# AI4Science-WestlakeU/safediffcon

Measured on AMD Instinct MI355X. Metric: sampled control trajectories/sec (1000-step DDPM), higher is better.
Workload: dtype f32; 1 GPU; C4: 2D smoke Unet3D_with_Conv3D dim=64 (1,2,4) state (B,32,7,64,64), B=64 per GPU, guided 1000-step DDPM, conformal quantile on; batch_per_gpu=64, global_batch=64, step=U-Net + guidance + posterior update of the whole batch, one hipGraph replay, parallelism=batch-sharded x1, no data-path collective, conv_precision=fp32

## Files before the change

### include/sdc.h

```cpp
#ifndef SDC_H
#define SDC_H

#include <stddef.h>
#include <stdint.h>

#ifdef __cplusplus
extern "C" {
#endif

#define SDC_OK 0
#define SDC_EINVAL (-1)
#define SDC_EALIGN (-2)
#define SDC_EHIP (-3)
#define SDC_ENULL (-4)

int sdc_version(void);
int sdc_last_error(char* buf, size_t cap);

typedef struct SdcConvDesc {
    int32_t B, Cin0, Cin1, Cout;
    int32_t iD, iH, iW;
    int32_t oD, oH, oW;
    int32_t kD, kH, kW;
    int32_t sD, sH, sW;
    int32_t pD, pH, pW;
    int32_t uD, uH, uW;
    int32_t up_mode;
    int32_t precision;
    int64_t x0s[5], x1s[5], ys[5], rs[5];
} SdcConvDesc;

int sdc_conv(const SdcConvDesc* d, const float* x0, const float* x1, const float* wp, const float* bias,
             const float* residual, float* y, void* stream);

size_t sdc_conv_splitk_bytes(const SdcConvDesc* d);
int sdc_conv_splitk(const SdcConvDesc* d, const float* x0, const float* x1, const float* wp, const float* bias, float* y,
                    float* work, size_t work_bytes, void* stream);

int sdc_conv_describe(const SdcConvDesc* d, char* name, size_t cap, double* mfma_share);

int sdc_conv_gnparts(const SdcConvDesc* d, int G);
int sdc_conv_gn(const SdcConvDesc* d, const float* x0, const float* x1, const float* wp, const float* bias,
                const float* residual, float* y, double* parts, int G, void* stream);

int sdc_gn_stats(const float* x, float* stats, int B, int C, int G, int64_t S, float eps, void* stream);
size_t sdc_gn_stats_bytes(int B, int G);
int sdc_gn_finalize(const double* parts, float* stats, int B, int G, int nparts, int64_t n_per_group, float eps, void* stream);

int sdc_gn_apply(const float* x, const float* stats, const float* gamma, const float* beta, const float* ss,
                 const int32_t* t_dev, int64_t ss_t_stride, int64_t ss_b_stride, int64_t ss_off,
                 const float* residual, float* y, int B, int C, int G, int64_t S, void* stream);

int sdc_gn_fused_ok(int B, int C, int G, int64_t S);
int sdc_gn_fused(const float* x, const float* gamma, const float* beta, const float* ss, const int32_t* t_dev,
                 int64_t ss_t_stride, int64_t ss_b_stride, int64_t ss_off, const float* residual, float* y, int B, int C, int G,
                 int64_t S, float eps, void* stream);

int sdc_gn_pointwise_out(const float* h, const float* stats, const float* gamma, const float* beta, const float* residual,
                         const float* w, const float* bias, float* y, int B, int C, int G, int Cout, int64_t S, int64_t plane,
                         int64_t ys0, int64_t ys1, int64_t ys2, void* stream);

int sdc_chan_norm(const float* x, const float* g, const float* residual, float* y, int B, int C, int64_t S,
                  int mode, float eps, void* stream);

int sdc_linattn(const float* qkv, float* ctx, float* out, int outer, int inner, int heads, int64_t n,
                int64_t q_so, int64_t q_sc, int64_t q_si, int64_t o_so, int64_t o_sc, int64_t o_si, void* stream);

size_t sdc_linattn_block_bytes(int outer, int inner, int C, int64_t n);
int sdc_linattn_block(const float* x, const float* g_pre, const float* wqkv, const float* wo, const float* bo,
                      const float* g_post, float* work, float* y, int outer, int inner, int C, int64_t n,
                      int64_t so, int64_t sc, int64_t si, int pre_mode, int post_mode, float eps, void* stream);
int sdc_linattn_block_gn(const float* x_raw, const float* gn_stats, const float* gn_gamma, const float* gn_beta, int gn_G,
                         const float* gn_residual, const float* g_pre, const float* wqkv, const float* wo, const float* bo,
                         const float* g_post, float* work, float* y, int outer, int inner, int C, int64_t n,
                         int64_t so, int64_t sc, int64_t si, int pre_mode, int post_mode, float eps, void* stream);

int sdc_tattn_block(const float* x, const float* g_pre, const float* wqkv, const float* wo, const float* rot,
                    const float* bias, float* y, int outer, int inner, int C, int ntok, int64_t so, int64_t sc,
                    int64_t st, float eps, void* stream);

size_t sdc_pack_tattn_f16_bytes(void);
int sdc_pack_tattn_f16(const float* wqkv, const float* wo, void* dst, void* stream);
int sdc_tattn_block_f16(const float* x, const float* g_pre, const void* wpk, const float* rot, const float* bias, float* y,
                        int outer, int inner, int C, int ntok, int64_t so, int64_t sc, int64_t st, float eps, void* stream);

int sdc_attn(const float* qkv, float* out, const float* rot, const float* bias, int outer, int inner, int heads,
             int ntok, int64_t q_so, int64_t q_sc, int64_t q_si, int64_t q_st,
             int64_t o_so, int64_t o_sc, int64_t o_si, int64_t o_st, void* stream);

int sdc_act(const float* x, float* y, int64_t n, int kind, void* stream);

#define SDC_MODEL_BURGERS 0
#define SDC_MODEL_TOKAMAK 1
#define SDC_MODEL_SMOKE 2

typedef struct SdcStepDesc {
    int32_t model;
    int32_t B;
    int32_t d0, d1, d2, d3;
    int32_t guide;
    int32_t clip;
    int32_t impose;
    int32_t cond_idx;
    int32_t pad_zero;
    int32_t use_max;
    int32_t has_wgt;
    int32_t skip_draws;
    int32_t ddim;
    uint64_t seed;
} SdcStepDesc;

int sdc_guide_reduce(const SdcStepDesc* d, const float* x, const float* eps, const float* coef, const int32_t* t_dev,
                     const float* gpar, float* gscal, void* stream);
int sdc_step_update(const SdcStepDesc* d, const float* x, const float* eps, const float* gext, const float* coef,
                    const int32_t* t_dev, const int32_t* draw_dev, const float* noise, int64_t noise_stride,
                    const float* gpar, const float* gscal, const float* target, const float* c0, const float* c1,
                    const float* c2, float* xout, float* x0out, void* stream);
int sdc_impose(const SdcStepDesc* d, float* x, const float* c0, const float* c1, const float* c2, void* stream);
int sdc_randn(float* x, int64_t n, uint64_t seed, const int32_t* draw_dev, void* stream);
int sdc_advance(int32_t* t_dev, int dt, int32_t* draw_dev, int ddraw, void* stream);

int sdc_advance_table(int32_t* idx_dev, int32_t* t_dev, const int32_t* ttab, int32_t* draw_dev, int ddraw, void* stream);

int sdc_conformal_score(const SdcStepDesc* d, const float* pred, const float* truth, const float* target,
                        const float* gpar, float* score, float* weight, void* stream);

int sdc_burgers_rollout(const float* u0, const float* f, float* traj, int N, int s, int Nt, int steps, int record_every,
                        float dt, float coef_transport, float d0, float d1, float d2, void* stream);


typedef struct SdcWgradDesc {
    int32_t B, M, N;
    int32_t oD, oH, oW;
    int32_t iD, iH, iW;
    int32_t kD, kH, kW;
    int32_t sD, sH, sW;
    int32_t pD, pH, pW;
    int32_t uD, uH, uW;
    int32_t precision;
    int64_t gs[5], xs[5];
} SdcWgradDesc;
size_t sdc_conv_wgrad_bytes(const SdcWgradDesc* d);
int sdc_conv_wgrad(const SdcWgradDesc* d, const float* g, const float* x, float* dw, float* dbias, void* work,
                   size_t work_bytes, void* stream);

#define SDC_F16_EXP_INTS 1025
int sdc_f16_grad_exponent(const float* g, int B, int C, int D, int H, int W, const int64_t* strides, int32_t* e, void* stream);

int sdc_conv_dgrad_f16(const SdcConvDesc* d, const float* g, const float* wp, const int32_t* e, float* dx, void* stream);

size_t sdc_conv_wgrad_f16_bytes(const SdcWgradDesc* d);
int sdc_conv_wgrad_f16(const SdcWgradDesc* d, const float* g, const float* x, const int32_t* e, float* dw, float* dbias, void* work,
                       size_t work_bytes, void* stream);
int sdc_conv_wgrad_describe(const SdcWgradDesc* d, char* name, size_t cap);

int sdc_conv_stem_f16_ok(const SdcConvDesc* d);
size_t sdc_pack_stem_f16_bytes(int Cout, int Cin, int kD, int kH, int kW);
int sdc_pack_stem_f16(const float* w, void* out, int Cout, int Cin, int kD, int kH, int kW, void* stream);
int sdc_conv_stem_f16(const SdcConvDesc* d, const float* x, const void* wh, const float* bias, float* y, void* stream);

int sdc_conv_stem_x3_ok(const SdcConvDesc* d);
size_t sdc_pack_stem_x3_bytes(int Cout, int Cin, int kD, int kH, int kW);
int sdc_pack_stem_x3(const float* w, void* out, int Cout, int Cin, int kD, int kH, int kW, void* stream);
int sdc_conv_stem_x3(const SdcConvDesc* d, const float* x, const void* wb, const float* bias, float* y, void* stream);

int sdc_conv_gemm_x3_ok(const SdcConvDesc* d);
size_t sdc_pack_gemm_x3_bytes(int Cout, int Cin, int kH, int kW);
int sdc_pack_gemm_x3(const float* wp, void* out, int Cout, int Cin, int kH, int kW, void* stream);
int sdc_conv_gemm_x3(const SdcConvDesc* d, const float* x, const void* wb, const float* bias, float* y, void* stream);

size_t sdc_gn_silu_bwd_floats(int B, int C, int G, int64_t S);
int sdc_gn_silu_bwd(const float* h, const float* gy, const float* stats, const float* gamma, const float* beta,
                    const float* ss, int64_t ss_b_stride, float* rows, float* gh, float* dgamma, float* dbeta, float* dss,
                    int B, int C, int G, int64_t S, void* stream);

size_t sdc_chan_norm_bwd_parts(int B, int64_t S);
size_t sdc_chan_norm_bwd_bytes(int B, int C, int64_t S);
int sdc_chan_norm_bwd(const float* x, const float* gy, const float* g, float* gx, float* gpart, int B, int C, int64_t S,
                      int mode, float eps, void* stream);

size_t sdc_pack_conv_weight_floats(int Cout, int Cin, int kD, int kH, int kW, int precision);
int sdc_pack_conv_weight(const float* w, float* out, int Cout, int Cin, int kD, int kH, int kW, int precision, int flip, void* stream);

typedef struct SdcPackItem {
    const float* w;
    float* out;
    int Cout, Cin, kD, kH, kW, precision, flip;
    int co_sh, ci_sh, grid_x, grid_y, block0;
    unsigned tap_magic;
    int64_t n[5];
} SdcPackItem;
int sdc_pack_batch_plan(SdcPackItem* items, int n, int* total_blocks, int* lds_bytes);
int sdc_pack_batch_run(const SdcPackItem* items_dev, int n, int total_blocks, int lds_bytes, void* stream);

size_t sdc_attn_bwd_bytes(int outer, int inner, int heads, int ntok);
int sdc_attn_bwd(const float* qkv, const float* dout, const float* rot, const float* bias, float* dqkv, float* dbias, void* work,
                 int outer, int inner, int heads, int ntok, int64_t q_so, int64_t q_sc, int64_t q_si, int64_t q_st,
                 int64_t o_so, int64_t o_sc, int64_t o_si, int64_t o_st, void* stream);
size_t sdc_linattn_bwd_bytes(int outer, int inner, int heads, int64_t n);
int sdc_linattn_bwd(const float* qkv, const float* dout, float* dqkv, void* work, int outer, int inner, int heads, int64_t n,
                    int64_t q_so, int64_t q_sc, int64_t q_si, int64_t o_so, int64_t o_sc, int64_t o_si, void* stream);

int sdc_act_bwd(const float* x, const float* gy, float* gx, int64_t n, int kind, void* stream);

int sdc_sumpool2(const float* g, float* gx, int64_t rows, int H, int W, int fh, int fw, void* stream);

int sdc_linear(const float* x, const float* w, const float* bias, float* y, int rows, int K, int M, int64_t x_stride,
               int64_t y_stride, void* stream);
int sdc_linear_dgrad(const float* gy, const float* w, float* gx, int rows, int K, int M, int64_t gy_stride, int64_t gx_stride,
                     void* stream);
int sdc_linear_wgrad(const float* gy, const float* x, float* gw, float* gbias, int rows, int K, int M, int64_t gy_stride,
                     int64_t x_stride, void* stream);

typedef struct {
    const void* ptr;
    int64_t nwords;
} SdcSpan;
int sdc_checksum_spans(const SdcSpan* spans_dev, int n, uint64_t* out_dev, void* stream);

#define SDC_OPT_SGD 0
#define SDC_OPT_ADAM 1
#define SDC_OPT_ADAMW 2
#define SDC_OPT_CLIP 1
#define SDC_OPT_SKIP_NONFINITE 2
#define SDC_OPT_HP_LR 0
#define SDC_OPT_HP_BETA1 1
#define SDC_OPT_HP_BETA2 2
#define SDC_OPT_HP_EPS 3
#define SDC_OPT_HP_WEIGHT_DECAY 4
#define SDC_OPT_HP_MAX_GRAD_NORM 5
#define SDC_OPT_HP_EMA_BETA 6
#define SDC_OPT_HP_EMA_UPDATE_EVERY 7
#define SDC_OPT_HP_EMA_UPDATE_AFTER_STEP 8
#define SDC_OPT_HP_COUNT 9
typedef struct SdcOptItem {
    float* p;
    const float* g;
    float* m;
    float* v;
    float* ema;
    int64_t n;
    int64_t chunk0;
} SdcOptItem;
typedef struct SdcOptState {
    int64_t step;
    float grad_norm;
    float clip_coef;
    int applied;
    int ema_mode;
} SdcOptState;
int sdc_optim_plan(SdcOptItem* items, int n, int kind, int* chunk, int* total_chunks, int* grid);
size_t sdc_optim_bytes(int total_chunks);
int sdc_optim_step(int kind, const SdcOptItem* items_dev, int n, int chunk, int total_chunks, int grid, const double* hp_dev,
                   SdcOptState* state_dev, void* work, int flags, void* stream);

int sdc_graph_begin(void* stream);
int sdc_graph_end(void* stream, void** graph_exec);
int sdc_graph_launch(void* graph_exec, void* stream);
int sdc_graph_destroy(void* graph_exec);

int sdc_event_create(void** ev);
int sdc_event_record(void* ev, void* stream);
int sdc_event_elapsed_ms(void* ev0, void* ev1, float* ms);
int sdc_event_destroy(void* ev);

#define SDC_KSTAR_SEQ 10
#define SDC_KSTAR_NIN 18
#define SDC_KSTAR_UNITS 100
typedef struct {
    int nlayers;
    int width[7];
    int act[6];
    const float* params;
    int64_t stride;
} SdcKstarMlp;
typedef struct {
    int n_lstm, n_bpw;
    const float* lstm;
    int64_t lstm_stride;
    SdcKstarMlp head;
    SdcKstarMlp steady;
    SdcKstarMlp bpw;
    double lstm_ystd[4], lstm_ymean[4], nn_ystd[4], nn_ymean[4], bpw_ystd[2], bpw_ymean[2];
    double scale;
    double inputs0[15];
    double low_action[9], high_action[9];
    double year_in;
} SdcKstarModel;
size_t sdc_kstar_lstm_floats(void);
int sdc_kstar_rollout(const SdcKstarModel* m, const float* actions, int64_t act_b_stride, int64_t act_t_stride,
                      int64_t act_c_stride, double* out, double* work, int B, int nsteps, void* stream);

size_t sdc_smoke_rollout_workspace_bytes(int B);
int sdc_smoke_rollout(const float* c1, const float* c2, int64_t ctrl_b_stride, int64_t ctrl_f_stride,
                      const float* init_density, int64_t dens_b_stride, const float* init_velocity, int64_t vel_b_stride,
                      const unsigned char* fluid_mask, const unsigned char* bucket_labels, const unsigned char* safe_labels,
                      int n_buckets, int n_safe, double* out, double* out_zero, void* work, size_t work_bytes, int B, int nt,
                      int nx, int per_timelength, int ring_lo, int ring_hi, double accuracy, int max_iterations, void* stream);

#ifdef __cplusplus
}
#endif
#endif
```

### safediffcon_amd/_lib.py

```python
import ctypes as C
import os

_HERE = os.path.dirname(os.path.abspath(__file__))
LIB_PATH = os.path.join(_HERE, "libsdc_hip.so")

SDC_MODEL_BURGERS, SDC_MODEL_TOKAMAK, SDC_MODEL_SMOKE = 0, 1, 2

_f32p = C.c_void_p
_i32p = C.c_void_p
_stream = C.c_void_p
_i64 = C.c_int64


class SdcConvDesc(C.Structure):
    _fields_ = [(n, C.c_int32) for n in (
        "B", "Cin0", "Cin1", "Cout", "iD", "iH", "iW", "oD", "oH", "oW", "kD", "kH", "kW", "sD", "sH", "sW",
        "pD", "pH", "pW", "uD", "uH", "uW", "up_mode", "precision")] + [
        ("x0s", C.c_int64 * 5), ("x1s", C.c_int64 * 5), ("ys", C.c_int64 * 5), ("rs", C.c_int64 * 5)]


class SdcStepDesc(C.Structure):
    _fields_ = [(n, C.c_int32) for n in (
        "model", "B", "d0", "d1", "d2", "d3", "guide", "clip", "impose", "cond_idx", "pad_zero", "use_max",
        "has_wgt", "skip_draws", "ddim")] + [("_pad", C.c_int32), ("seed", C.c_uint64)]


class SdcWgradDesc(C.Structure):
    _fields_ = [(n, C.c_int32) for n in (
        "B", "M", "N", "oD", "oH", "oW", "iD", "iH", "iW", "kD", "kH", "kW", "sD", "sH", "sW", "pD", "pH", "pW",
        "uD", "uH", "uW", "precision")] + [("gs", C.c_int64 * 5), ("xs", C.c_int64 * 5)]


class SdcPackItem(C.Structure):
    _fields_ = [("w", C.c_void_p), ("out", C.c_void_p)] + [(n, C.c_int32) for n in (
        "Cout", "Cin", "kD", "kH", "kW", "precision", "flip", "co_sh", "ci_sh", "grid_x", "grid_y", "block0")] + [
        ("tap_magic", C.c_uint32), ("_pad", C.c_int32), ("n", C.c_int64 * 5)]


class SdcOptItem(C.Structure):
    _fields_ = [("p", C.c_void_p), ("g", C.c_void_p), ("m", C.c_void_p), ("v", C.c_void_p), ("ema", C.c_void_p),
                ("n", C.c_int64), ("chunk0", C.c_int64)]


class SdcOptState(C.Structure):
    _fields_ = [("step", C.c_int64), ("grad_norm", C.c_float), ("clip_coef", C.c_float), ("applied", C.c_int32), ("ema_mode", C.c_int32)]


class SdcSpan(C.Structure):
    _fields_ = [("ptr", C.c_void_p), ("nwords", C.c_int64)]


class SdcKstarMlp(C.Structure):
    _fields_ = [("nlayers", C.c_int32), ("width", C.c_int32 * 7), ("act", C.c_int32 * 6), ("params", C.c_void_p), ("stride", C.c_int64)]


class SdcKstarModel(C.Structure):
    _fields_ = [("n_lstm", C.c_int32), ("n_bpw", C.c_int32), ("lstm", C.c_void_p), ("lstm_stride", C.c_int64),
                ("head", SdcKstarMlp), ("steady", SdcKstarMlp), ("bpw", SdcKstarMlp),
                ("lstm_ystd", C.c_double * 4), ("lstm_ymean", C.c_double * 4), ("nn_ystd", C.c_double * 4), ("nn_ymean", C.c_double * 4),
                ("bpw_ystd", C.c_double * 2), ("bpw_ymean", C.c_double * 2), ("scale", C.c_double), ("inputs0", C.c_double * 15),
                ("low_action", C.c_double * 9), ("high_action", C.c_double * 9), ("year_in", C.c_double)]


SIGNATURES = {
    "sdc_version": (C.c_int, []),
    "sdc_last_error": (C.c_int, [C.c_char_p, C.c_size_t]),
    "sdc_conv": (C.c_int, [C.POINTER(SdcConvDesc), _f32p, _f32p, _f32p, _f32p, _f32p, _f32p, _stream]),
    "sdc_conv_describe": (C.c_int, [C.POINTER(SdcConvDesc), C.c_char_p, C.c_size_t, C.POINTER(C.c_double)]),
    "sdc_conv_gnparts": (C.c_int, [C.POINTER(SdcConvDesc), C.c_int]),
    "sdc_conv_gn": (C.c_int, [C.POINTER(SdcConvDesc), _f32p, _f32p, _f32p, _f32p, _f32p, _f32p, C.c_void_p, C.c_int, _stream]),
    "sdc_gn_finalize": (C.c_int, [C.c_void_p, _f32p, C.c_int, C.c_int, C.c_int, _i64, C.c_float, _stream]),
    "sdc_gn_stats": (C.c_int, [_f32p, _f32p, C.c_int, C.c_int, C.c_int, _i64, C.c_float, _stream]),
    "sdc_gn_stats_bytes": (C.c_size_t, [C.c_int, C.c_int]),
    "sdc_gn_apply": (C.c_int, [_f32p, _f32p, _f32p, _f32p, _f32p, _i32p, _i64, _i64, _i64, _f32p, _f32p,
                               C.c_int, C.c_int, C.c_int, _i64, _stream]),
    "sdc_gn_fused_ok": (C.c_int, [C.c_int, C.c_int, C.c_int, _i64]),
    "sdc_gn_fused": (C.c_int, [_f32p, _f32p, _f32p, _f32p, _i32p, _i64, _i64, _i64, _f32p, _f32p, C.c_int, C.c_int, C.c_int, _i64,
                               C.c_float, _stream]),
    "sdc_gn_pointwise_out": (C.c_int, [_f32p, _f32p, _f32p, _f32p, _f32p, _f32p, _f32p, _f32p, C.c_int, C.c_int, C.c_int, C.c_int, _i64,
                                       _i64, _i64, _i64, _i64, _stream]),
    "sdc_chan_norm": (C.c_int, [_f32p, _f32p, _f32p, _f32p, C.c_int, C.c_int, _i64, C.c_int, C.c_float, _stream]),
    "sdc_linattn": (C.c_int, [_f32p, _f32p, _f32p, C.c_int, C.c_int, C.c_int, _i64, _i64, _i64, _i64, _i64, _i64,
                              _i64, _stream]),
    "sdc_linattn_block_bytes": (C.c_size_t, [C.c_int, C.c_int, C.c_int, _i64]),
    "sdc_linattn_block": (C.c_int, [_f32p, _f32p, _f32p, _f32p, _f32p, _f32p, _f32p, _f32p, C.c_int, C.c_int, C.c_int, _i64,
                                    _i64, _i64, _i64, C.c_int, C.c_int, C.c_float, _stream]),
    "sdc_linattn_block_gn": (C.c_int, [_f32p, _f32p, _f32p, _f32p, C.c_int, _f32p, _f32p, _f32p, _f32p, _f32p, _f32p, _f32p, _f32p,
                                       C.c_int, C.c_int, C.c_int, _i64, _i64, _i64, _i64, C.c_int, C.c_int, C.c_float, _stream]),
    "sdc_tattn_block": (C.c_int, [_f32p, _f32p, _f32p, _f32p, _f32p, _f32p, _f32p, C.c_int, C.c_int, C.c_int, C.c_int,
                                  _i64, _i64, _i64, C.c_float, _stream]),
    "sdc_pack_tattn_f16_bytes": (C.c_size_t, []),
    "sdc_pack_tattn_f16": (C.c_int, [_f32p, _f32p, C.c_void_p, _stream]),
    "sdc_tattn_block_f16": (C.c_int, [_f32p, _f32p, C.c_void_p, _f32p, _f32p, _f32p, C.c_int, C.c_int, C.c_int, C.c_int,
                                      _i64, _i64, _i64, C.c_float, _stream]),
    "sdc_attn": (C.c_int, [_f32p, _f32p, _f32p, _f32p, C.c_int, C.c_int, C.c_int, C.c_int, _i64, _i64, _i64, _i64,
                           _i64, _i64, _i64, _i64, _stream]),
    "sdc_act": (C.c_int, [_f32p, _f32p, _i64, C.c_int, _stream]),
    "sdc_guide_reduce": (C.c_int, [C.POINTER(SdcStepDesc), _f32p, _f32p, _f32p, _i32p, _f32p, _f32p, _stream]),
    "sdc_step_update": (C.c_int, [C.POINTER(SdcStepDesc), _f32p, _f32p, _f32p, _f32p, _i32p, _i32p, _f32p, _i64,
                                  _f32p, _f32p, _f32p, _f32p, _f32p, _f32p, _f32p, _f32p, _stream]),
    "sdc_impose": (C.c_int, [C.POINTER(SdcStepDesc), _f32p, _f32p, _f32p, _f32p, _stream]),
    "sdc_randn": (C.c_int, [_f32p, _i64, C.c_uint64, _i32p, _stream]),
    "sdc_advance": (C.c_int, [_i32p, C.c_int, _i32p, C.c_int, _stream]),
    "sdc_advance_table": (C.c_int, [_i32p, _i32p, _i32p, _i32p, C.c_int, _stream]),
    "sdc_conformal_score": (C.c_int, [C.POINTER(SdcStepDesc), _f32p, _f32p, _f32p, _f32p, _f32p, _f32p, _stream]),
    "sdc_burgers_rollout": (C.c_int, [_f32p, _f32p, _f32p, C.c_int, C.c_int, C.c_int, C.c_int, C.c_int, C.c_float, C.c_float,
                                      C.c_float, C.c_float, C.c_float, _stream]),
    "sdc_conv_wgrad_bytes": (C.c_size_t, [C.POINTER(SdcWgradDesc)]),
    "sdc_conv_wgrad": (C.c_int, [C.POINTER(SdcWgradDesc), _f32p, _f32p, _f32p, _f32p, C.c_void_p, C.c_size_t, _stream]),
    "sdc_f16_grad_exponent": (C.c_int, [_f32p, C.c_int, C.c_int, C.c_int, C.c_int, C.c_int, C.c_void_p, C.c_void_p, _stream]),
    "sdc_conv_dgrad_f16": (C.c_int, [C.POINTER(SdcConvDesc), _f32p, _f32p, C.c_void_p, _f32p, _stream]),
    "sdc_conv_stem_f16_ok": (C.c_int, [C.POINTER(SdcConvDesc)]),
    "sdc_pack_stem_f16_bytes": (C.c_size_t, [C.c_int, C.c_int, C.c_int, C.c_int, C.c_int]),
    "sdc_pack_stem_f16": (C.c_int, [_f32p, C.c_void_p, C.c_int, C.c_int, C.c_int, C.c_int, C.c_int, _stream]),
    "sdc_conv_stem_f16": (C.c_int, [C.POINTER(SdcConvDesc), _f32p, C.c_void_p, _f32p, _f32p, _stream]),
    "sdc_conv_stem_x3_ok": (C.c_int, [C.POINTER(SdcConvDesc)]),
    "sdc_pack_stem_x3_bytes": (C.c_size_t, [C.c_int, C.c_int, C.c_int, C.c_int, C.c_int]),
    "sdc_pack_stem_x3": (C.c_int, [_f32p, C.c_void_p, C.c_int, C.c_int, C.c_int, C.c_int, C.c_int, _stream]),
    "sdc_conv_stem_x3": (C.c_int, [C.POINTER(SdcConvDesc), _f32p, C.c_void_p, _f32p, _f32p, _stream]),
    "sdc_conv_gemm_x3_ok": (C.c_int, [C.POINTER(SdcConvDesc)]),
    "sdc_pack_gemm_x3_bytes": (C.c_size_t, [C.c_int, C.c_int, C.c_int, C.c_int]),
    "sdc_pack_gemm_x3": (C.c_int, [_f32p, C.c_void_p, C.c_int, C.c_int, C.c_int, C.c_int, _stream]),
    "sdc_conv_gemm_x3": (C.c_int, [C.POINTER(SdcConvDesc), _f32p, C.c_void_p, _f32p, _f32p, _stream]),
    "sdc_conv_wgrad_f16_bytes": (C.c_size_t, [C.POINTER(SdcWgradDesc)]),
    "sdc_conv_wgrad_f16": (C.c_int, [C.POINTER(SdcWgradDesc), _f32p, _f32p, C.c_void_p, _f32p, _f32p, C.c_void_p, C.c_size_t, _stream]),
    "sdc_conv_wgrad_describe": (C.c_int, [C.POINTER(SdcWgradDesc), C.c_char_p, C.c_size_t]),
    "sdc_gn_silu_bwd_floats": (C.c_size_t, [C.c_int, C.c_int, C.c_int, _i64]),
    "sdc_gn_silu_bwd": (C.c_int, [_f32p, _f32p, _f32p, _f32p, _f32p, _f32p, _i64, _f32p, _f32p, _f32p, _f32p, _f32p,
                                  C.c_int, C.c_int, C.c_int, _i64, _stream]),
    "sdc_chan_norm_bwd_parts": (C.c_size_t, [C.c_int, _i64]),
    "sdc_chan_norm_bwd_bytes": (C.c_size_t, [C.c_int, C.c_int, _i64]),
    "sdc_chan_norm_bwd": (C.c_int, [_f32p, _f32p, _f32p, _f32p, _f32p, C.c_int, C.c_int, _i64, C.c_int, C.c_float, _stream]),
    "sdc_pack_conv_weight_floats": (C.c_size_t, [C.c_int, C.c_int, C.c_int, C.c_int, C.c_int, C.c_int]),
    "sdc_pack_conv_weight": (C.c_int, [_f32p, _f32p, C.c_int, C.c_int, C.c_int, C.c_int, C.c_int, C.c_int, C.c_int, _stream]),
    "sdc_pack_batch_plan": (C.c_int, [C.POINTER(SdcPackItem), C.c_int, C.POINTER(C.c_int), C.POINTER(C.c_int)]),
    "sdc_pack_batch_run": (C.c_int, [C.c_void_p, C.c_int, C.c_int, C.c_int, _stream]),
    "sdc_attn_bwd_bytes": (C.c_size_t, [C.c_int, C.c_int, C.c_int, C.c_int]),
    "sdc_attn_bwd": (C.c_int, [_f32p, _f32p, _f32p, _f32p, _f32p, _f32p, C.c_void_p, C.c_int, C.c_int, C.c_int, C.c_int,
                               _i64, _i64, _i64, _i64, _i64, _i64, _i64, _i64, _stream]),
    "sdc_linattn_bwd_bytes": (C.c_size_t, [C.c_int, C.c_int, C.c_int, _i64]),
    "sdc_linattn_bwd": (C.c_int, [_f32p, _f32p, _f32p, C.c_void_p, C.c_int, C.c_int, C.c_int, _i64, _i64, _i64, _i64, _i64, _i64, _i64,
                                  _stream]),
    "sdc_act_bwd": (C.c_int, [_f32p, _f32p, _f32p, _i64, C.c_int, _stream]),
    "sdc_sumpool2": (C.c_int, [_f32p, _f32p, _i64, C.c_int, C.c_int, C.c_int, C.c_int, _stream]),
    "sdc_kstar_lstm_floats": (C.c_size_t, []),
    "sdc_kstar_rollout": (C.c_int, [C.POINTER(SdcKstarModel), _f32p, _i64, _i64, _i64, C.c_void_p, C.c_void_p, C.c_int, C.c_int, _stream]),
    "sdc_smoke_rollout_workspace_bytes": (C.c_size_t, [C.c_int]),
    "sdc_smoke_rollout": (C.c_int, [_f32p, _f32p, _i64, _i64, _f32p, _i64, _f32p, _i64, C.c_void_p, C.c_void_p, C.c_void_p,
                                    C.c_int, C.c_int, C.c_void_p, C.c_void_p, C.c_void_p, C.c_size_t, C.c_int, C.c_int, C.c_int,
                                    C.c_int, C.c_int, C.c_int, C.c_double, C.c_int, _stream]),
    "sdc_conv_splitk_bytes": (C.c_size_t, [C.POINTER(SdcConvDesc)]),
    "sdc_conv_splitk": (C.c_int, [C.POINTER(SdcConvDesc), _f32p, _f32p, _f32p, _f32p, _f32p, _f32p, C.c_size_t, _stream]),
    "sdc_linear": (C.c_int, [_f32p, _f32p, _f32p, _f32p, C.c_int, C.c_int, C.c_int, _i64, _i64, _stream]),
    "sdc_linear_dgrad": (C.c_int, [_f32p, _f32p, _f32p, C.c_int, C.c_int, C.c_int, _i64, _i64, _stream]),
    "sdc_linear_wgrad": (C.c_int, [_f32p, _f32p, _f32p, _f32p, C.c_int, C.c_int, C.c_int, _i64, _i64, _stream]),
    "sdc_checksum_spans": (C.c_int, [C.c_void_p, C.c_int, C.c_void_p, _stream]),
    "sdc_optim_plan": (C.c_int, [C.POINTER(SdcOptItem), C.c_int, C.c_int, C.POINTER(C.c_int), C.POINTER(C.c_int), C.POINTER(C.c_int)]),
    "sdc_optim_bytes": (C.c_size_t, [C.c_int]),
    "sdc_optim_step": (C.c_int, [C.c_int, C.c_void_p, C.c_int, C.c_int, C.c_int, C.c_int, C.c_void_p, C.c_void_p, C.c_void_p, C.c_int,
                                 _stream]),
    "sdc_graph_begin": (C.c_int, [_stream]),
    "sdc_graph_end": (C.c_int, [_stream, C.POINTER(C.c_void_p)]),
    "sdc_graph_launch": (C.c_int, [C.c_void_p, _stream]),
    "sdc_graph_destroy": (C.c_int, [C.c_void_p]),
    "sdc_event_create": (C.c_int, [C.POINTER(C.c_void_p)]),
    "sdc_event_record": (C.c_int, [C.c_void_p, _stream]),
    "sdc_event_elapsed_ms": (C.c_int, [C.c_void_p, C.c_void_p, C.POINTER(C.c_float)]),
    "sdc_event_destroy": (C.c_int, [C.c_void_p]),
}

_lib = None


class SdcError(RuntimeError):
    pass


def use_library(path):
    global LIB_PATH
    if _lib is not None:
        raise SdcError("use_library() after the library has been loaded")
    LIB_PATH = os.path.abspath(path)


def get_lib():
    global _lib
    if _lib is None:
        if not os.path.exists(LIB_PATH):
            raise SdcError(
                f"{LIB_PATH} not found: build it with `python -m safediffcon_amd.build` "
                "(hipcc --offload-arch=gfx950). safediffcon_amd has no CPU/eager fallback.")
        lib = C.CDLL(LIB_PATH)
        for name, (res, args) in SIGNATURES.items():
            fn = getattr(lib, name)
            fn.restype, fn.argtypes = res, args
        _lib = lib
    return _lib


def last_error():
    buf = C.create_string_buffer(512)
    get_lib().sdc_last_error(buf, 512)
    return buf.value.decode(errors="replace")


def check(rc, what=""):
    if rc != 0:
        raise SdcError(f"{what or 'libsdc_hip'} failed (code {rc}): {last_error()}")
```

### safediffcon_amd/build.py

```python
import os
import subprocess
import sys

HERE = os.path.dirname(os.path.abspath(__file__))
CSRC = os.path.join(HERE, "csrc")
LIB = os.path.join(HERE, "libsdc_hip.so")
SOURCES = ["sdc_api.hip", "sdc_conv.hip", "sdc_conv_wino.hip", "sdc_conv_f16.hip", "sdc_conv_stem_f16.hip", "sdc_conv_stem_x3.hip", "sdc_conv_gemm_x3.hip", "sdc_norm.hip", "sdc_attn.hip", "sdc_lablock.hip", "sdc_tablock.hip", "sdc_tablock_f16.hip", "sdc_step.hip", "sdc_solver.hip", "sdc_grad.hip", "sdc_wgrad_f16.hip", "sdc_attn_bwd.hip", "sdc_kstar.hip", "sdc_smoke.hip", "sdc_linear.hip", "sdc_optim.hip"]
HEADERS = ["sdc_common.h", "sdc_conv.h", "sdc_conv_wino3s.inc", "sdc_conv_wino2s.inc", "sdc_conv_pw2.inc"]
HIPCC = os.environ.get("HIPCC", "/opt/rocm/bin/hipcc")
FLAGS = ["--offload-arch=gfx950", "-O3", "-fPIC", "-std=c++17", "-Wall", "-Wno-unused-function"]


def source_hash():
    import hashlib
    h = hashlib.sha256()
    for f in SOURCES + HEADERS:
        with open(os.path.join(CSRC, f), "rb") as fh:
            h.update(fh.read())
    with open(os.path.join(HERE, "..", "include", "sdc.h"), "rb") as fh:
        h.update(fh.read())
    return h.hexdigest()[:16]


def _stale(out, deps):
    if not os.path.exists(out):
        return True
    t = os.path.getmtime(out)
    return any(os.path.getmtime(d) > t for d in deps)


def build_experiments(verbose=True):
    out = os.path.join(HERE, "libsdc_hip_exp.so")
    cmd = [HIPCC, *FLAGS, "-DSDC_KERNEL_EXPERIMENTS", "-shared", *[os.path.join(CSRC, s) for s in SOURCES], "-o", out]
    if verbose:
        print(" ".join(cmd), flush=True)
    subprocess.check_call(cmd)
    return out


def build(force=False, verbose=True, jobs=4):
    from concurrent.futures import ThreadPoolExecutor
    hdrs = [os.path.join(CSRC, h) for h in HEADERS] + [os.path.join(HERE, "..", "include", "sdc.h")]
    objs, todo = [], []
    for src in SOURCES:
        s = os.path.join(CSRC, src)
        o = os.path.join(CSRC, src.replace(".hip", ".o"))
        if force or _stale(o, [s] + hdrs):
            todo.append([HIPCC, *FLAGS, "-c", s, "-o", o])
        objs.append(o)

    def run(cmd):
        if verbose:
            print(" ".join(cmd), flush=True)
        subprocess.check_call(cmd)
    if todo:
        with ThreadPoolExecutor(max_workers=max(1, min(jobs, len(todo)))) as ex:
            list(ex.map(run, todo))
    if force or _stale(LIB, objs):
        run([HIPCC, "--offload-arch=gfx950", "-shared", "-fPIC", *objs, "-o", LIB])
    return LIB


if __name__ == "__main__":
    if "--experiments" in sys.argv:
        build_experiments()
    else:
        build(force="--force" in sys.argv)
```

### safediffcon_amd/engine.py

```python
import ctypes as C
import functools
import os
import math

import torch

from . import _lib
from ._lib import SdcConvDesc, check


def _ptr(t):
    return 0 if t is None else t.data_ptr()


def _s5(t):
    assert t.dim() == 5, t.shape
    return tuple(int(s) for s in t.stride())


def as5(t):
    while t.dim() < 5:
        t = t.unsqueeze(2)
    return t


@functools.lru_cache(maxsize=16)
def _up2_merge(parity, device):
    return torch.tensor([[1, 0, 0], [0, 1, 1]] if parity == 0 else [[1, 1, 0], [0, 0, 1]], dtype=torch.float64, device=device)


def pack_conv_weight(t, kind="conv", precision=0):
    def base():
        if kind == "convT":
            t5 = as5(t)
            t5 = t5.flip(2, 3, 4).permute(2, 3, 4, 0, 1)
            return t5.reshape(-1, t5.shape[-1]).contiguous()
        if isinstance(kind, tuple) and kind[0] == "convT_sub":
            _, ph, pw = kind
            t5 = as5(t)
            kh = (3, 1) if ph == 0 else (2, 0)
            kw = (3, 1) if pw == 0 else (2, 0)
            sub = t5[:, :, 0][:, :, (1 - ph)::2][:, :, :, (1 - pw)::2].flip(2, 3)
            assert kh == ((3, 1) if ph == 0 else (2, 0)) and kw == ((3, 1) if pw == 0 else (2, 0))
            return sub.permute(2, 3, 0, 1).reshape(-1, sub.shape[1]).contiguous()
        if isinstance(kind, tuple) and kind[0] == "up2_sub":
            _, ph, pw = kind
            t5 = as5(t).to(torch.float64)
            mh, mw = _up2_merge(ph, t5.device), _up2_merge(pw, t5.device)
            sub = torch.einsum("ah,bw,oihw->oiab", mh, mw, t5[:, :, 0])
            return sub.permute(2, 3, 1, 0).reshape(-1, sub.shape[0]).to(torch.float32).contiguous()
        if kind == "unshuffle":
            co, c4 = t.shape[0], t.shape[1]
            t4 = t.reshape(co, c4 // 4, 2, 2)
            return t4.permute(2, 3, 1, 0).reshape(-1, co).contiguous()
        t5 = as5(t)
        return t5.permute(2, 3, 4, 1, 0).reshape(-1, t5.shape[0]).contiguous()
    if precision in (6, 7):
        p4 = pack_conv_weight(t, kind, 4)
        k = tuple(as5(t).shape[2:])
        if kind != "conv" or f16_kc(k) == 0:
            return p4
        return torch.cat([p4, p4.new_zeros(-p4.numel() % 4), f16_tail(t)])
    wp = base().to(torch.float32)
    if precision not in (2, 3, 4, 5) or kind != "conv" or t.shape[-1] != 3:
        return wp
    t5 = as5(t).to(torch.float64)
    G = torch.tensor([[1, 0, 0], [.5, .5, .5], [.5, -.5, .5], [0, 0, 1]], dtype=torch.float64, device=t5.device)
    u = torch.einsum("xk,oidhk->dhxio", G, t5)
    parts = [wp.reshape(-1), u.reshape(-1).to(torch.float32)]
    if precision == 5 and t5.shape[2] == 1 and t5.shape[3] == 1:
        G43 = torch.tensor([[1 / 4, 0, 0], [-1 / 6, -1 / 6, -1 / 6], [-1 / 6, 1 / 6, -1 / 6], [1 / 24, 1 / 12, 1 / 6],
                            [1 / 24, -1 / 12, 1 / 6], [0, 0, 1]], dtype=torch.float64, device=t5.device)
        u43 = torch.einsum("xk,oik->xio", G43, t5[:, :, 0, 0])
        return torch.cat(parts + [u43.reshape(-1).to(torch.float32)])
    if precision >= 3 and t5.shape[3] == 3:
        u2 = torch.einsum("jh,xk,oidhk->diojx", G, G, t5)
        parts.append(u2.reshape(-1).to(torch.float32))
        if precision >= 4 and t5.shape[2] == 3:
            u3 = torch.einsum("zd,jh,xk,oidhk->ziojx", G, G, G, t5)
            parts.append(u3.reshape(-1).to(torch.float32))
    return torch.cat(parts)


def f16_kc(k):
    k = tuple(k)
    return 32 if tuple(k) in ((1, 1, 3), (1, 3, 3), (3, 3, 3)) else 0


def f16_tail(t, flip=False):
    t5 = as5(t).to(torch.float32)
    if flip:
        t5 = t5.transpose(0, 1).flip((2, 3, 4))
    co, ci = t5.shape[0], t5.shape[1]
    kc = f16_kc(t5.shape[2:])
    nch = (ci + kc - 1) // kc
    w = t5.permute(2, 3, 4, 1, 0).reshape(-1, ci, co)
    w = torch.cat([w, w.new_zeros(w.shape[0], nch * kc - ci, co)], 1)
    w = w.reshape(w.shape[0], nch, kc, co).permute(0, 1, 3, 2).contiguous()
    return w.half().reshape(-1).view(torch.float32)


def pack_stem_f16(w):
    t5 = as5(w).to(torch.float32)
    co, ci, kD, kH, kW = t5.shape
    if not (kW == 7 and (kD, kH) in ((1, 1), (1, 7), (7, 7)) and 1 <= ci <= 8):
        raise ValueError(f"pack_stem_f16: taps 1x1x7, 1x7x7 or 7x7x7 and Cin <= 8 (got {tuple(t5.shape)})")
    taps, ns = kH * 7, (kH * 7 + 1) // 2
    z = t5.new_zeros(co, 8, kD, 2 * ns)
    z[:, :ci, :, :taps] = t5.reshape(co, ci, kD, taps)
    z = z.reshape(co, 8, kD, ns, 2).permute(2, 3, 0, 4, 1).contiguous()
    return z.half().reshape(-1).view(torch.float32)


def pack_stem_x3(w):
    t5 = as5(w).to(torch.float32)
    co, ci, kD, kH, kW = t5.shape
    if not (kW == 7 and (kD, kH) in ((1, 1), (1, 7), (7, 7)) and 1 <= ci <= 8):
        raise ValueError(f"pack_stem_x3: taps 1x1x7, 1x7x7 or 7x7x7 and Cin <= 8 (got {tuple(t5.shape)})")
    taps, ns = kH * 7, (kH * 7 + 1) // 2
    z = t5.new_zeros(co, 8, kD, 2 * ns)
    z[:, :ci, :, :taps] = t5.reshape(co, ci, kD, taps)
    z = z.reshape(co, 8, kD, ns, 2).permute(2, 3, 0, 4, 1).contiguous()
    return torch.stack(split3_bf16(z)).reshape(-1).view(torch.float32)


def pack_tattn_f16(wqkv, wo):
    wqkv, wo = wqkv.to(torch.float32), wo.to(torch.float32)
    if tuple(wqkv.shape) != (384, 64) or tuple(wo.shape) != (64, 128):
        raise ValueError(f"pack_tattn_f16: to_qkv (384, 64) and to_out (64, 128) (got {tuple(wqkv.shape)}, {tuple(wo.shape)})")
    a = wqkv.reshape(3, 4, 32, 4, 2, 8).permute(1, 0, 3, 4, 2, 5)
    b = wo.reshape(2, 32, 4, 2, 2, 2, 4).permute(2, 0, 3, 5, 1, 4, 6)
    return torch.cat([a.reshape(-1), b.reshape(-1)]).half().view(torch.float32)


def pack_gemm_x3(wp, cout, cin, k):
    k = tuple(k)[-2:]
    ncb = {(4, 4): 1, (2, 2): 2, (1, 1): 4}.get(k, 0)
    taps = k[0] * k[1]
    if ncb == 0 or cout <= 0 or cout % 64 or cin <= 0 or cin % (16 * ncb) or tuple(wp.shape) != (taps * cin, cout):
        raise ValueError(f"pack_gemm_x3: taps 4x4, 2x2 or 1x1, Cout % 64 == 0, Cin % {16 * max(ncb, 1)} == 0, Wp [taps * Cin][Cout] "
                         f"(got taps {k}, Cin {cin}, Cout {cout}, Wp {tuple(wp.shape)})")
    z = wp.to(torch.float32).reshape(taps, cin // (16 * ncb), ncb, 16, cout // 64, 64)
    z = z.permute(4, 1, 2, 0, 5, 3).contiguous()
    return torch.stack(split3_bf16(z)).reshape(-1).view(torch.float32)


def split3_bf16(x):
    h = x.bfloat16()
    r = x - h.float()
    m = r.bfloat16()
    return h, m, (r - m.float()).bfloat16()


def conv_precision(n, k, cin, cout, f16=None, train=False):
    floats = functools.partial(_lib.get_lib().sdc_pack_conv_weight_floats, cout, cin, *k)
    if train:
        assert f16 in (6, 7) and n == floats(8), (f16, n, k, cin, cout)
        return f16
    if f16 in (6, 7) and f16_kc(k) > 0 and n == floats(6):
        return f16
    code = next((p for p in (0, 2, 3, 4, 5) if n == floats(p)), None)
    assert code is not None, (n, k, cin, cout)
    return code


def conv_desc(x, x1, out, residual, cout, k, stride, pad, up, up_mode, precision):
    d = SdcConvDesc()
    d.B, d.Cin0, d.iD, d.iH, d.iW = x.shape
    d.Cin1, d.Cout = (0 if x1 is None else x1.shape[1]), cout
    d.oD, d.oH, d.oW = out.shape[2:]
    d.kD, d.kH, d.kW = k
    d.sD, d.sH, d.sW = stride
    d.pD, d.pH, d.pW = pad
    d.uD, d.uH, d.uW = up
    d.up_mode, d.precision = up_mode, precision
    d.x0s[:] = _s5(x)
    d.x1s[:] = _s5(x1) if x1 is not None else (0,) * 5
    d.ys[:] = _s5(out)
    d.rs[:] = _s5(residual) if residual is not None else (0,) * 5
    return d


class Pool:

    def __init__(self, device):
        self.device = device
        self.free = {}
        self.all = []
        self.bytes = 0

    def get(self, shape):
        n = int(math.prod(shape))
        lst = self.free.get(n)
        if lst:
            return lst.pop().view(shape)
        t = torch.empty(n, dtype=torch.float32, device=self.device)
        self.all.append(t)
        self.bytes += n * 4
        return t.view(shape)

    def put(self, t):
        self.free.setdefault(t.numel(), []).append(t.reshape(-1))


class Plan:

    def __init__(self, device, precision=0, stem_f16=False, stem_split=False, gemm_split=False, attn_f16=False):
        self.device = torch.device(device)
        self.lib = _lib.get_lib()
        self.precision = int(precision)
        if self.precision not in (0, 2, 3, 4, 5, 6, 7):
            raise ValueError(f"precision must be 0, 2, 3, 4, 5, 6 or 7 (got {precision})")
        self.stem_f16 = bool(stem_f16)
        self.stem_split = bool(stem_split) and self.precision >= 4 and not self.stem_f16
        self.gemm_split = bool(gemm_split) and self.precision >= 4
        self.attn_f16 = bool(attn_f16)
        self.calls = []
        self.pool = Pool(self.device)
        self.keep = []
        self.repackers = []
        self._stats = None
        self._ctx = None
        self._gn_parts = {}
        self.fuse_gn_stats = True
        self.fuse_gn_small = True
        self.split_small_grids = False

    def run(self, stream):
        for fn, args in self.calls:
            rc = fn(*args, stream)
            if rc:
                check(rc, fn.__name__)

    def refresh_weights(self):
        with torch.no_grad():
            for dst, fn in self.repackers:
                dst.copy_(fn())

    def _stats_buf(self, B, G):
        need = int(self.lib.sdc_gn_stats_bytes(B, G))
        if self._stats is None or self._stats.numel() * 4 < need:
            self._stats = torch.empty((need + 3) // 4, dtype=torch.float32, device=self.device)
            self.keep.append(self._stats)
        return self._stats

    def _ctx_buf(self, n):
        if self._ctx is None or self._ctx.numel() < n:
            self._ctx = torch.empty(n, dtype=torch.float32, device=self.device)
            self.keep.append(self._ctx)
        return self._ctx

    def _emit(self, fn, *args):
        self.calls.append((fn, args))

    def packed(self, src_fn):
        with torch.no_grad():
            w = src_fn().detach().to(self.device, torch.float32).contiguous().clone()
        self.repackers.append((w, lambda: src_fn().detach().to(self.device, torch.float32)))
        self.keep.append(w)
        return w

    def conv_weight(self, w, kind="conv"):
        return self.packed(lambda: pack_conv_weight(w() if callable(w) else w, kind, self.precision))

    def stem_weight(self, w, pack=pack_stem_f16):
        return self.packed(lambda: pack(w() if callable(w) else w))

    def vec(self, p):
        return self.packed(lambda: (p() if callable(p) else p).reshape(-1))

    def conv(self, x, wp, bias, cout, k, *, x1=None, stride=(1, 1, 1), pad=(0, 0, 0), up=(1, 1, 1), up_mode=0,
             residual=None, out=None, gn_groups=0, stem_w=None, gemm_w=None):
        B, c0, iD, iH, iW = x.shape
        c1 = 0 if x1 is None else x1.shape[1]

        def osz(i, u, kk, s, p):
            v = (i - 1) * u + 1 if up_mode else i * u
            return (v + 2 * p - kk) // s + 1

        o = tuple(osz(i, u, kk, s, p) for i, u, kk, s, p in zip((iD, iH, iW), up, k, stride, pad))
        if out is None:
            out = self.pool.get((B, cout, *o))
        else:
            assert tuple(out.shape[:2]) == (B, cout) and out.dim() == 5, (out.shape, (B, cout, *o))
            o = tuple(out.shape[2:])
        if (self.stem_f16 or self.stem_split) and stem_w is not None and x1 is None and residual is None:
            d = conv_desc(x, None, out, None, cout, k, stride, pad, up, up_mode, 0)
            ok, fn, pack = ((self.lib.sdc_conv_stem_f16_ok, self.lib.sdc_conv_stem_f16, pack_stem_f16) if self.stem_f16 else
                            (self.lib.sdc_conv_stem_x3_ok, self.lib.sdc_conv_stem_x3, pack_stem_x3))
            if ok(C.byref(d)):
                wh = self.stem_weight(stem_w, pack)
                self.keep += [d, x, wh, bias, out]
                self._emit(fn, C.byref(d), _ptr(x), _ptr(wh), _ptr(bias), _ptr(out))
                return out
        if self.gemm_split and gemm_w is not None and x1 is None and residual is None and not gn_groups:
            d = conv_desc(x, None, out, None, cout, k, stride, pad, up, up_mode, 0)
            if self.lib.sdc_conv_gemm_x3_ok(C.byref(d)) and not (self.split_small_grids and self.lib.sdc_conv_splitk_bytes(C.byref(d))):
                wb = self.packed(lambda: pack_gemm_x3(gemm_w(), cout, c0, k))
                self.keep += [d, x, wb, bias, out]
                self._emit(self.lib.sdc_conv_gemm_x3, C.byref(d), _ptr(x), _ptr(wb), _ptr(bias), _ptr(out))
                return out
        if callable(wp):
            wp = wp()
        prec = conv_precision(wp.numel(), k, c0 + c1, cout, f16=self.precision)
        d = conv_desc(x, x1, out, residual, cout, k, stride, pad, up, up_mode, prec)
        if residual is not None:
            assert tuple(residual.shape) == tuple(out.shape)
        self.keep += [d, x, x1, wp, bias, residual, out]
        if self.split_small_grids and residual is None:
            nsplit = int(self.lib.sdc_conv_splitk_bytes(C.byref(d)))
            if nsplit:
                work = torch.empty(nsplit // 4, dtype=torch.float32, device=self.device)
                self.keep.append(work)
                self._emit(self.lib.sdc_conv_splitk, C.byref(d), _ptr(x), _ptr(x1), _ptr(wp), _ptr(bias), _ptr(out), _ptr(work), nsplit)
                return out
        nparts = int(self.lib.sdc_conv_gnparts(C.byref(d), gn_groups)) if (gn_groups and self.fuse_gn_stats) else 0
        if nparts > 0:
            parts = torch.empty(B * gn_groups * nparts * 2, dtype=torch.float64, device=self.device)
            self.keep.append(parts)
            self._gn_parts[out.data_ptr()] = (parts, nparts, gn_groups)
            self._emit(self.lib.sdc_conv_gn, C.byref(d), _ptr(x), _ptr(x1), _ptr(wp), _ptr(bias), _ptr(residual), _ptr(out),
                       _ptr(parts), gn_groups)
            return out
        self._emit(self.lib.sdc_conv, C.byref(d), _ptr(x), _ptr(x1), _ptr(wp), _ptr(bias), _ptr(residual), _ptr(out))
        return out

    def conv_transpose_422(self, x, w, bias, cout):
        B, c0, iD, iH, iW = x.shape
        out = self.pool.get((B, cout, iD, 2 * iH, 2 * iW))
        for ph in (0, 1):
            for pw in (0, 1):
                kind = ("convT_sub", ph, pw)
                if self.gemm_split:
                    self.conv(x, lambda kind=kind: self.conv_weight(w, kind), bias, cout, (1, 2, 2), pad=(0, 1 - ph, 1 - pw),
                              out=out[:, :, :, ph::2, pw::2], gemm_w=lambda kind=kind: pack_conv_weight(w() if callable(w) else w, kind, 0))
                    continue
                wp = self.conv_weight(w, kind)
                self.conv(x, wp, bias, cout, (1, 2, 2), pad=(0, 1 - ph, 1 - pw), out=out[:, :, :, ph::2, pw::2])
        return out

    def upsample2_conv3(self, x, w, bias, cout):
        B, c0, iD, iH, iW = x.shape
        out = self.pool.get((B, cout, iD, 2 * iH, 2 * iW))
        for ph in (0, 1):
            for pw in (0, 1):
                wp = self.conv_weight(w, ("up2_sub", ph, pw))
                self.conv(x, wp, bias, cout, (1, 2, 2), pad=(0, 1 - ph, 1 - pw), out=out[:, :, :, ph::2, pw::2])
        return out

    def gn_silu(self, x, gamma, beta, groups, *, ss=None, t_dev=None, ss_t_stride=0, ss_b_stride=0, ss_off=0,
                residual=None, out=None, eps=1e-5):
        assert x.is_contiguous()
        B, Cc = x.shape[0], x.shape[1]
        S = x.numel() // (B * Cc)
        st = self._stats_buf(B, groups)
        out = x if out is None else out
        self.keep += [x, gamma, beta, ss, t_dev, residual, out]
        fused = self._gn_parts.pop(x.data_ptr(), None)
        if fused is not None and fused[2] == groups:
            self._emit(self.lib.sdc_gn_finalize, _ptr(fused[0]), _ptr(st), B, groups, fused[1], (Cc // groups) * S, eps)
        elif self.fuse_gn_small and self.lib.sdc_gn_fused_ok(B, Cc, groups, S):
            self._emit(self.lib.sdc_gn_fused, _ptr(x), _ptr(gamma), _ptr(beta), _ptr(ss), _ptr(t_dev), ss_t_stride, ss_b_stride,
                       ss_off, _ptr(residual), _ptr(out), B, Cc, groups, S, eps)
            return out
        else:
            self._emit(self.lib.sdc_gn_stats, _ptr(x), _ptr(st), B, Cc, groups, S, eps)
        self._emit(self.lib.sdc_gn_apply, _ptr(x), _ptr(st), _ptr(gamma), _ptr(beta), _ptr(ss), _ptr(t_dev),
                   ss_t_stride, ss_b_stride, ss_off, _ptr(residual), _ptr(out), B, Cc, groups, S)
        return out

    def chan_norm(self, x, g, mode, *, residual=None, out=None, eps=1e-5):
        assert x.is_contiguous()
        B, Cc = x.shape[0], x.shape[1]
        S = x.numel() // (B * Cc)
        if out is None:
            out = self.pool.get(tuple(x.shape))
        self.keep += [x, g, residual, out]
        self._emit(self.lib.sdc_chan_norm, _ptr(x), _ptr(g), _ptr(residual), _ptr(out), B, Cc, S, mode, eps)
        return out

    def act(self, x, kind, out=None):
        out = x if out is None else out
        self.keep += [x, out]
        self._emit(self.lib.sdc_act, _ptr(x), _ptr(out), x.numel(), kind)
        return out

    def linattn(self, qkv, heads, outer, inner, n, q_strides, out, o_strides):
        ctx = self._ctx_buf(outer * inner * heads * 32 * 32)
        self.keep += [qkv, out]
        self._emit(self.lib.sdc_linattn, _ptr(qkv), _ptr(ctx), _ptr(out), outer, inner, heads, n, *q_strides, *o_strides)
        return out

    def gn_stats_deferred(self, x, groups, eps=1e-5):
        assert x.is_contiguous()
        B, Cc = x.shape[0], x.shape[1]
        S = x.numel() // (B * Cc)
        st = torch.empty((int(self.lib.sdc_gn_stats_bytes(B, groups)) + 3) // 4, dtype=torch.float32, device=self.device)
        self.keep += [x, st]
        fused = self._gn_parts.pop(x.data_ptr(), None)
        if fused is not None and fused[2] == groups:
            self._emit(self.lib.sdc_gn_finalize, _ptr(fused[0]), _ptr(st), B, groups, fused[1], (Cc // groups) * S, eps)
        else:
            self._emit(self.lib.sdc_gn_stats, _ptr(x), _ptr(st), B, Cc, groups, S, eps)
        return st

    def gn_apply_deferred(self, x, gn):
        st, gamma, beta, groups, res = gn
        B, Cc = x.shape[0], x.shape[1]
        S = x.numel() // (B * Cc)
        self.keep += [x, st, gamma, beta, res]
        self._emit(self.lib.sdc_gn_apply, _ptr(x), _ptr(st), _ptr(gamma), _ptr(beta), 0, 0, 0, 0, 0, _ptr(res), _ptr(x), B, Cc, groups, S)
        return x

    def gn_pointwise_out(self, x, gn, w, bias, out):
        st, gamma, beta, groups, res = gn
        B, Cc = x.shape[0], x.shape[1]
        S = x.numel() // (B * Cc)
        cout = out.shape[1]
        plane = out.shape[3] * out.shape[4]
        ys = _s5(out)
        ok = (x.is_contiguous() and (res is None or res.is_contiguous()) and cout <= 16 and Cc % 4 == 0 and Cc <= 2048 and S >= 1024 and plane % 4 == 0 and ys[4] == 1 and
              ys[3] == out.shape[4] and all(v % 4 == 0 for v in ys[:3]) and out.data_ptr() % 16 == 0 and
              tuple(out.shape[2:]) == tuple(x.shape[2:]))
        if not ok:
            return None
        self.keep += [x, st, gamma, beta, res, w, bias, out]
        self._emit(self.lib.sdc_gn_pointwise_out, _ptr(x), _ptr(st), _ptr(gamma), _ptr(beta), _ptr(res), _ptr(w), _ptr(bias), _ptr(out),
                   B, Cc, groups, cout, S, plane, ys[0], ys[1], ys[2])
        return out

    def linattn_block(self, x, g_pre, wqkv, wo, bo, g_post, outer, inner, n, strides, pre_mode, post_mode, eps=1e-5, gn=None):
        Cc = x.shape[1]
        y = self.pool.get(tuple(x.shape))
        work = torch.empty(int(self.lib.sdc_linattn_block_bytes(outer, inner, Cc, n)) // 4, dtype=torch.float32, device=self.device)
        self.keep += [x, g_pre, wqkv, wo, bo, g_post, work, y]
        if gn is not None:
            st, gamma, beta, groups, res = gn
            assert outer == x.shape[0] and (res is None or (tuple(res.shape) == tuple(x.shape) and res.stride() == x.stride()))
            self.keep += [st, gamma, beta, res]
            self._emit(self.lib.sdc_linattn_block_gn, _ptr(x), _ptr(st), _ptr(gamma), _ptr(beta), groups, _ptr(res), _ptr(g_pre),
                       _ptr(wqkv), _ptr(wo), _ptr(bo), _ptr(g_post), _ptr(work), _ptr(y), outer, inner, Cc, n, *strides, pre_mode,
                       post_mode, eps)
            return y
        self._emit(self.lib.sdc_linattn_block, _ptr(x), _ptr(g_pre), _ptr(wqkv), _ptr(wo), _ptr(bo), _ptr(g_post), _ptr(work),
                   _ptr(y), outer, inner, Cc, n, *strides, pre_mode, post_mode, eps)
        return y

    def tattn_weight(self, wqkv, wo):
        return self.packed(lambda: pack_tattn_f16(wqkv() if callable(wqkv) else wqkv, wo() if callable(wo) else wo))

    def tattn_block(self, x, g_pre, wqkv, wo, rot, bias, eps=1e-5):
        B, Cc, Fr, H, W = x.shape
        assert x.is_contiguous()
        y = self.pool.get(tuple(x.shape))
        if self.attn_f16:
            wpk = self.tattn_weight(wqkv, wo)
            self.keep += [x, g_pre, wpk, rot, bias, y]
            self._emit(self.lib.sdc_tattn_block_f16, _ptr(x), _ptr(g_pre), _ptr(wpk), _ptr(rot), _ptr(bias), _ptr(y),
                       B, H * W, Cc, Fr, Cc * Fr * H * W, Fr * H * W, H * W, eps)
            return y
        self.keep += [x, g_pre, wqkv, wo, rot, bias, y]
        self._emit(self.lib.sdc_tattn_block, _ptr(x), _ptr(g_pre), _ptr(wqkv), _ptr(wo), _ptr(rot), _ptr(bias), _ptr(y),
                   B, H * W, Cc, Fr, Cc * Fr * H * W, Fr * H * W, H * W, eps)
        return y

    def attn(self, qkv, out, heads, outer, inner, ntok, q_strides, o_strides, rot=None, bias=None):
        self.keep += [qkv, out, rot, bias]
        self._emit(self.lib.sdc_attn, _ptr(qkv), _ptr(out), _ptr(rot), _ptr(bias), outer, inner, heads, ntok,
                   *q_strides, *o_strides)
        return out
```

### safediffcon_amd/unet.py

```python
import ctypes as C
import functools
import math
import os

import torch
from torch import nn

from ._lib import check, get_lib
from .engine import Plan, as5, pack_conv_weight

HEADS, DIM_HEAD = 4, 32
HID = HEADS * DIM_HEAD


def _resnet_spec(p, cin, cout, time_dim, k):
    s = []
    if time_dim is not None:
        s += [(f"{p}.mlp.1.weight", (cout * 2, time_dim)), (f"{p}.mlp.1.bias", (cout * 2,))]
    for blk, ci in (("block1", cin), ("block2", cout)):
        s += [(f"{p}.{blk}.proj.weight", (cout, ci, *k)), (f"{p}.{blk}.proj.bias", (cout,)),
              (f"{p}.{blk}.norm.weight", (cout,)), (f"{p}.{blk}.norm.bias", (cout,))]
    if cin != cout:
        s += [(f"{p}.res_conv.weight", (cout, cin, *([1] * len(k)))), (f"{p}.res_conv.bias", (cout,))]
    return s


def spec_lucid(dim, dim_mults, channels, nd):
    one, k3, k7 = [1] * nd, [3] * nd, [7] * nd
    g = (1, 0, *one)
    td = dim * 4
    dims = [dim] + [dim * m for m in dim_mults]
    io = list(zip(dims[:-1], dims[1:]))
    gshape = lambda c: (1, c, *one)
    s = []
    if nd == 1:
        s += [("init_conv.weight", (dim, channels, *k7)), ("init_conv.bias", (dim,))]
    s += [("time_mlp.1.weight", (td, dim)), ("time_mlp.1.bias", (td,)),
          ("time_mlp.3.weight", (td, td)), ("time_mlp.3.bias", (td,))]
    if nd == 2:
        s += [("init_conv.weight", (dim, channels, *k7)), ("init_conv.bias", (dim,))]

    def lin_attn(p, c):
        return [(f"{p}.fn.fn.to_qkv.weight", (HID * 3, c, *one)), (f"{p}.fn.fn.to_out.0.weight", (c, HID, *one)),
                (f"{p}.fn.fn.to_out.0.bias", (c,)), (f"{p}.fn.fn.to_out.1.g", gshape(c)), (f"{p}.fn.norm.g", gshape(c))]

    def full_attn(p, c):
        return [(f"{p}.fn.fn.to_qkv.weight", (HID * 3, c, *one)), (f"{p}.fn.fn.to_out.weight", (c, HID, *one)),
                (f"{p}.fn.fn.to_out.bias", (c,)), (f"{p}.fn.norm.g", gshape(c))]

    downs, ups = [], []
    for i, (ci, co) in enumerate(io):
        last = i == len(io) - 1
        p = f"downs.{i}"
        downs += _resnet_spec(f"{p}.0", ci, ci, td, k3) + _resnet_spec(f"{p}.1", ci, ci, td, k3) + lin_attn(f"{p}.2", ci)
        if last:
            downs += [(f"{p}.3.weight", (co, ci, *k3)), (f"{p}.3.bias", (co,))]
        elif nd == 2:
            downs += [(f"{p}.3.1.weight", (co, ci * 4, *one)), (f"{p}.3.1.bias", (co,))]
        else:
            downs += [(f"{p}.3.weight", (co, ci, 4)), (f"{p}.3.bias", (co,))]
    mid = dims[-1]
    mids = _resnet_spec("mid_block1", mid, mid, td, k3) + full_attn("mid_attn", mid) + _resnet_spec("mid_block2", mid, mid, td, k3)
    for i, (ci, co) in enumerate(reversed(io)):
        last = i == len(io) - 1
        p = f"ups.{i}"
        ups += _resnet_spec(f"{p}.0", co + ci, co, td, k3) + _resnet_spec(f"{p}.1", co + ci, co, td, k3) + lin_attn(f"{p}.2", co)
        if last:
            ups += [(f"{p}.3.weight", (ci, co, *k3)), (f"{p}.3.bias", (ci,))]
        else:
            ups += [(f"{p}.3.1.weight", (ci, co, *k3)), (f"{p}.3.1.bias", (ci,))]
    fin = _resnet_spec("final_res_block", dim * 2, dim, td, k3) + [("final_conv.weight", (channels, dim, *one)),
                                                                   ("final_conv.bias", (channels,))]
    if nd == 2:
        return s + downs + mids + ups + fin
    return s + downs + ups + mids + fin


def spec_smoke(dim, dim_mults, channels):
    td = dim * 4
    dims = [dim] + [dim * m for m in dim_mults]
    io = list(zip(dims[:-1], dims[1:]))
    k3, one = (3, 3, 3), (1, 1, 1)
    rot = ("rotary_emb.freqs", (DIM_HEAD // 2,))

    def t_attn(p, c):
        return [(f"{p}.fn.fn.fn.{rot[0]}", rot[1]), (f"{p}.fn.fn.fn.to_qkv.weight", (HID * 3, c)),
                (f"{p}.fn.fn.fn.to_out.weight", (c, HID)), (f"{p}.fn.norm.gamma", (1, c, 1, 1, 1))]

    def s_lin(p, c):
        return [(f"{p}.fn.fn.to_qkv.weight", (HID * 3, c, 1, 1)), (f"{p}.fn.fn.to_out.weight", (c, HID, 1, 1)),
                (f"{p}.fn.fn.to_out.bias", (c,)), (f"{p}.fn.norm.gamma", (1, c, 1, 1, 1))]

    s = [("time_rel_pos_bias.relative_attention_bias.weight", (32, HEADS)),
         ("init_conv.weight", (dim, channels, 7, 7, 7)), ("init_conv.bias", (dim,))]
    s += t_attn("init_temporal_attn", dim)
    s += [("time_mlp.1.weight", (td, dim)), ("time_mlp.1.bias", (td,)), ("time_mlp.3.weight", (td, td)),
          ("time_mlp.3.bias", (td,))]
    downs, ups = [], []
    for i, (ci, co) in enumerate(io):
        p = f"downs.{i}"
        downs += _resnet_spec(f"{p}.0", ci, co, td, k3) + _resnet_spec(f"{p}.1", co, co, td, k3) + s_lin(f"{p}.2", co) + t_attn(f"{p}.3", co)
        if i < len(io) - 1:
            downs += [(f"{p}.4.weight", (co, co, 1, 4, 4)), (f"{p}.4.bias", (co,))]
    for i, (ci, co) in enumerate(reversed(io)):
        p = f"ups.{i}"
        ups += _resnet_spec(f"{p}.0", co * 2, ci, td, k3) + _resnet_spec(f"{p}.1", ci, ci, td, k3) + s_lin(f"{p}.2", ci) + t_attn(f"{p}.3", ci)
        if i < len(io) - 1:
            ups += [(f"{p}.4.weight", (ci, ci, 1, 4, 4)), (f"{p}.4.bias", (ci,))]
    mid = dims[-1]
    mids = _resnet_spec("mid_block1", mid, mid, td, k3)
    mids += [("mid_spatial_attn.fn.fn.fn.to_qkv.weight", (HID * 3, mid)), ("mid_spatial_attn.fn.fn.fn.to_out.weight", (mid, HID)),
             ("mid_spatial_attn.fn.norm.gamma", (1, mid, 1, 1, 1))]
    mids += t_attn("mid_temporal_attn", mid) + _resnet_spec("mid_block2", mid, mid, td, k3)
    fin = _resnet_spec("final_conv.0", dim * 2, dim, None, k3) + [("final_conv.1.weight", (channels, dim, *one)),
                                                                 ("final_conv.1.bias", (channels,))]
    return s + downs + ups + mids + fin


def _register(root, key, value):
    *mods, leaf = key.split(".")
    m = root
    for name in mods:
        if name not in m._modules:
            m.add_module(name, nn.Module())
        m = m._modules[name]
    m.register_parameter(leaf, nn.Parameter(value))


def _default_init(spec, gen):
    out = {}
    for key, shape in spec:
        leaf = key.rsplit(".", 1)[-1]
        if key.endswith("rotary_emb.freqs"):
            d = 2 * shape[0]
            v = 1.0 / (10000 ** (torch.arange(0, d, 2)[: d // 2].float() / d))
        elif key.endswith("relative_attention_bias.weight"):
            v = torch.randn(shape, generator=gen)
        elif leaf in ("g", "gamma") or key.endswith("norm.weight"):
            v = torch.ones(shape)
        elif key.endswith("norm.bias"):
            v = torch.zeros(shape)
        else:
            wshape = shape if leaf != "bias" else None
            if wshape is None:
                wkey = key[: -len("bias")] + "weight"
                wshape = dict(spec)[wkey]
            bound = 1.0 / math.sqrt(max(1, math.prod(wshape[1:])))
            v = (torch.rand(shape, generator=gen) * 2 - 1) * bound
        out[key] = v
    return out


def sinusoid_table(times, dim, theta=10000.0):
    return _sinusoid(times.detach().cpu(), dim, theta)


@functools.lru_cache(maxsize=32)
def _sinusoid_freqs(n, device, theta):
    return torch.exp(torch.arange(n) * -(math.log(theta) / (n - 1))).to(device)


def _sinusoid(t, dim, theta=10000.0):
    half = dim // 2
    f = _sinusoid_freqs(half, t.device, theta)
    a = t[:, None] * f[None, :]
    if dim % 2 == 0:
        return torch.cat((a.sin(), a.cos()), dim=-1)
    half1 = (dim + 1) // 2
    f1 = _sinusoid_freqs(half1, t.device, theta)
    return torch.cat((a.sin(), (t[:, None] * f1[None, :]).cos()), dim=-1)


class _Builder:

    def __init__(self, net, plan):
        self.net, self.plan = net, plan
        self.cond_sites = []

    def W(self, key, kind="conv"):
        return self.plan.conv_weight(lambda: self.net.P(key), kind)

    def V(self, key):
        return self.plan.vec(lambda: self.net.P(key))

    def ksize(self, key):
        shp = tuple(self.net.P(key).shape[2:])
        return (1,) * (3 - len(shp)) + shp

    def conv(self, x, prefix, *, x1=None, stride=1, pad=None, up=(1, 1, 1), residual=None, out=None, kind="conv",
             bias=True, gn_groups=0):
        wkey = f"{prefix}.weight"
        w = self.net.P(wkey)
        if kind == "convT":
            cout, k = w.shape[1], self.ksize(wkey)
        elif kind == "unshuffle":
            cout, k = w.shape[0], (1, 2, 2)
        else:
            cout, k = w.shape[0], self.ksize(wkey)
        if isinstance(stride, int):
            stride = tuple(stride if kk > 1 else 1 for kk in k)
        if pad is None:
            pad = tuple(kk // 2 for kk in k)
        b = self.V(f"{prefix}.bias") if bias else None
        if (self.plan.stem_f16 or self.plan.stem_split) and kind == "conv" and k[2] == 7:
            return self.plan.conv(x, lambda: self.W(wkey, kind), b, cout, k, x1=x1, stride=stride, pad=pad, up=up, residual=residual,
                                  out=out, gn_groups=gn_groups, stem_w=lambda: self.net.P(wkey))
        if self.plan.gemm_split and kind == "conv" and k in ((1, 4, 4), (1, 1, 1)) and x1 is None and residual is None:
            return self.plan.conv(x, lambda: self.W(wkey, kind), b, cout, k, stride=stride, pad=pad, up=up, out=out, gn_groups=gn_groups,
                                  gemm_w=lambda: pack_conv_weight(self.net.P(wkey), kind, 0))
        return self.plan.conv(x, self.W(wkey, kind), b, cout, k, x1=x1, stride=stride, pad=pad, up=up,
                              up_mode=1 if kind == "convT" else 0, residual=residual, out=out, gn_groups=gn_groups)

    def final_conv(self, res_prefix, conv_prefix, h, groups, x1, out):
        pool = self.plan.pool
        if self.net.fuse_final_conv and h.shape[2] * h.shape[3] * h.shape[4] >= 1024:
            g, gn, rbuf = self.resnet(res_prefix, h, groups, x1=x1, defer_gn=True)
            wv, bv = self.V(f"{conv_prefix}.weight"), self.V(f"{conv_prefix}.bias")
            if self.plan.gn_pointwise_out(g, gn, wv, bv, out) is not None:
                pool.put(g)
                if rbuf is not None:
                    pool.put(rbuf)
                return
            self.plan.gn_apply_deferred(g, gn)
            if rbuf is not None:
                pool.put(rbuf)
            f = g
        else:
            f = self.resnet(res_prefix, h, groups, x1=x1)
        self.conv(f, conv_prefix, out=out)
        pool.put(f)

    def gn(self, x, prefix, groups, residual=None, cond_off=None):
        self.plan.gn_silu(x, self.V(f"{prefix}.weight"), self.V(f"{prefix}.bias"), groups, residual=residual)
        if cond_off is not None:
            self.cond_sites.append((len(self.plan.calls) - 1, cond_off))

    def resnet(self, prefix, x, groups, *, x1=None, defer_gn=False):
        net, pool = self.net, self.plan.pool
        h = self.conv(x, f"{prefix}.block1.proj", x1=x1, gn_groups=groups)
        self.gn(h, f"{prefix}.block1.norm", groups, cond_off=net.cond_offsets.get(prefix))
        g = self.conv(h, f"{prefix}.block2.proj", gn_groups=groups)
        pool.put(h)
        own = net.has(f"{prefix}.res_conv.weight")
        if own:
            r = self.conv(x, f"{prefix}.res_conv", x1=x1)
        else:
            assert x1 is None
            r = x
        if defer_gn:
            st = self.plan.gn_stats_deferred(g, groups)
            return g, (st, self.V(f"{prefix}.block2.norm.weight"), self.V(f"{prefix}.block2.norm.bias"), groups, r), (r if own else None)
        self.gn(g, f"{prefix}.block2.norm", groups, residual=r)
        if own:
            pool.put(r)
        return g


class _HipUNet(nn.Module):

    def __init__(self, spec, dim, seed=None):
        super().__init__()
        gen = torch.Generator()
        gen.manual_seed(int(torch.initial_seed()) & 0x7FFFFFFF if seed is None else seed)
        for k, v in _default_init(spec, gen).items():
            _register(self, k, v)
        self._spec = spec
        self._plans = {}
        self.precision = 4
        self.train_precision = None
        self.stem_f16 = False
        self.attn_f16 = False
        self.stem_split = True
        self.gemm_split = True
        self.fuse_linattn = True
        self.fuse_gn_into_linattn = True
        self.content_stamp = True
        self.subpixel_upsample = True
        self.split_small_grids = False
        self.fuse_final_conv = True
        self.forward_graph = True
        self._side = None
        self.dim = dim
        self.self_condition = False
        self.cond_offsets, off = {}, 0
        for k, shape in spec:
            if k.endswith(".mlp.1.weight"):
                self.cond_offsets[k[: -len(".mlp.1.weight")]] = off
                off += shape[0]
        self.cond_width = off

    @property
    def train_precision(self):
        return self.__dict__.get("_train_precision")

    @train_precision.setter
    def train_precision(self, v):
        from .autograd import check_train_precision
        self.__dict__["_train_precision"] = check_train_precision(v)

    def P(self, key):
        m = self
        *mods, leaf = key.split(".")
        for name in mods:
            m = m._modules[name]
        return m._parameters[leaf]

    def has(self, key):
        try:
            return self.P(key) is not None
        except KeyError:
            return False

    def _trainer(self):
        if getattr(self, "_train_ctx", None) is None:
            from .autograd import Trainer
            self._train_ctx = Trainer(self)
        return self._train_ctx

    def forward_train(self, x, time):
        if not x.is_cuda:
            raise RuntimeError("safediffcon_amd runs on MI355X only: tensors must be on a cuda (HIP) device; "
                               "there is no CPU fallback")
        from . import autograd
        fn = autograd.forward_train_smoke if isinstance(self, Unet3D_with_Conv3D) else autograd.forward_train_lucid
        with self._trainer().step(x.device):
            return fn(self, x.to(torch.float32), time)

    def _drop_plans(self):
        self._train_ctx = None
        for e in self._plans.values():
            g = e.get("graph")
            if g is not None:
                torch.cuda.synchronize(e["x"].device)
                e["plan"].lib.sdc_graph_destroy(g)
                e["graph"] = None
        self._plans = {}
        self._side = None

    def _apply(self, fn, *a, **k):
        self._drop_plans()
        return super()._apply(fn, *a, **k)

    def load_state_dict(self, sd, strict=True, **kw):
        sd = {k: v for k, v in sd.items() if ("rotary_emb." not in k) or k.endswith("rotary_emb.freqs")}
        r = super().load_state_dict(sd, strict=strict, **kw)
        self.refresh()
        return r

    def _stamp_tensors(self):
        return [t for t in list(self.parameters()) + list(self.buffers()) if t.is_cuda and t.numel() and t.element_size() == 4]

    def _content_stamp(self):
        ts = self._stamp_tensors()
        if not ts:
            return 0
        from ._lib import SdcSpan
        dev = ts[0].device
        key = tuple((t.data_ptr(), t.numel()) for t in ts)
        tab = getattr(self, "_span_tab", None)
        if tab is None or tab[0] != key:
            arr = (SdcSpan * len(ts))(*[SdcSpan(t.data_ptr(), t.numel()) for t in ts])
            host = torch.frombuffer(bytearray(bytes(arr)), dtype=torch.uint8)
            tab = self._span_tab = (key, host.to(dev), torch.zeros(1, dtype=torch.int64, device=dev))
        lib = get_lib()
        check(lib.sdc_checksum_spans(tab[1].data_ptr(), len(ts), tab[2].data_ptr(), torch.cuda.current_stream(dev).cuda_stream),
              "sdc_checksum_spans")
        return int(tab[2].item())

    def _weights_stamp(self):
        host = hash(tuple((p.data_ptr(), p._version) for p in self.parameters()))
        dev = next(self.parameters()).device
        if not (self.content_stamp and dev.type == "cuda"):
            return (host, 0)
        if torch.cuda.is_current_stream_capturing():
            return (host, getattr(self, "_last_content", 0))
        self._last_content = self._content_stamp()
        return (host, self._last_content)

    def _refresh_entry(self, e, stamp):
        e["plan"].refresh_weights()
        e["cond"].refresh_weights()
        e["lut_valid"] = False
        e["wstamp"] = stamp

    def refresh(self):
        stamp = self._weights_stamp()
        for e in self._plans.values():
            self._refresh_entry(e, stamp)

    def device(self):
        return next(self.parameters()).device

    def entry(self, shape, rows, lut=False):
        key = (tuple(shape), rows, bool(lut), int(self.precision), bool(self.fuse_linattn), bool(self.subpixel_upsample),
               bool(self.fuse_gn_into_linattn), bool(self.split_small_grids), bool(self.fuse_final_conv), bool(self.stem_f16),
               bool(self.stem_split), bool(self.gemm_split), bool(self.attn_f16))
        stamp = self._weights_stamp()
        ent = self._plans.get(key)
        if ent is not None and ent["wstamp"] != stamp:
            self._refresh_entry(ent, stamp)
        if key not in self._plans:
            dev = self.device()
            if dev.type != "cuda":
                raise RuntimeError("safediffcon_amd runs on MI355X only: move the model to a cuda (HIP) device; "
                                   "there is no CPU fallback")
            plan = Plan(dev, precision=self.precision, stem_f16=bool(self.stem_f16), stem_split=bool(self.stem_split),
                        gemm_split=bool(self.gemm_split), attn_f16=bool(self.attn_f16))
            plan.split_small_grids = bool(self.split_small_grids)
            x = torch.zeros(shape, dtype=torch.float32, device=dev)
            eps = torch.zeros(shape, dtype=torch.float32, device=dev)
            b = _Builder(self, plan)
            self._build(b, x, eps)
            plan.cond_sites = b.cond_sites
            cond = Plan(dev)
            td = self.dim * 4
            emb = torch.zeros((rows, self.dim, 1, 1, 1), dtype=torch.float32, device=dev)
            cb = _Builder(self, cond)
            h = cb.conv(emb, "time_mlp.1")
            cond.act(h, 1)
            temb = cb.conv(h, "time_mlp.3")
            cond.act(temb, 0)
            prefixes = list(self.cond_offsets)
            wcat = cond.conv_weight(lambda: torch.cat([self.P(f"{p}.mlp.1.weight") for p in prefixes], 0))
            bcat = cond.vec(lambda: torch.cat([self.P(f"{p}.mlp.1.bias") for p in prefixes], 0))
            ss = cond.conv(temb, wcat, bcat, self.cond_width, (1, 1, 1))
            assert temb.shape[1] == td
            self._plans[key] = dict(plan=plan, cond=cond, x=x, eps=eps, emb=emb, ss=ss, rows=rows, lut_valid=False,
                                    t_dev=None, wstamp=stamp)
        return self._plans[key]

    def bind_cond(self, ent, t_dev):
        plan, ss, W = ent["plan"], ent["ss"], self.cond_width
        for idx, off in plan.cond_sites:
            fn, a = plan.calls[idx]
            a = list(a)
            i0 = 3 if fn is plan.lib.sdc_gn_fused else 4
            if t_dev is None:
                a[i0:i0 + 5] = ss.data_ptr(), 0, 0, W, off
            else:
                a[i0:i0 + 5] = ss.data_ptr(), t_dev.data_ptr(), W, 0, off
            plan.calls[idx] = (fn, tuple(a))
        ent["t_dev"] = t_dev

    def fill_cond(self, ent, times, stream):
        ent["emb"].copy_(sinusoid_table(times, self.dim).reshape(ent["emb"].shape), non_blocking=False)
        ent["cond"].run(stream)

    def forward(self, x, time, x_self_cond=None, **unused):
        if not x.is_cuda:
            raise RuntimeError("safediffcon_amd runs on MI355X only: tensors must be on a cuda (HIP) device; "
                               "there is no CPU fallback")
        ent = self.entry(tuple(x.shape), x.shape[0])
        stream = torch.cuda.current_stream(x.device).cuda_stream
        with torch.no_grad():
            if not ent.get("bound"):
                self.bind_cond(ent, None)
                ent["bound"] = True
            ent["x"].copy_(x)
            emb = _sinusoid(time.detach().to(x.device), self.dim)
            ent["emb"].copy_(emb.reshape(ent["emb"].shape))
            if not self.forward_graph:
                ent["cond"].run(stream)
                ent["plan"].run(stream)
                return ent["eps"].clone()
            cur = torch.cuda.current_stream(x.device)
            if self._side is None or self._side.device != x.device:
                self._side = torch.cuda.Stream(x.device)
            side = self._side
            side.wait_stream(cur)
            lib = ent["plan"].lib
            if ent.get("graph") is None:
                check(lib.sdc_graph_begin(side.cuda_stream), "sdc_graph_begin")
                try:
                    ent["cond"].run(side.cuda_stream)
                    ent["plan"].run(side.cuda_stream)
                finally:
                    g = C.c_void_p()
                    rc = lib.sdc_graph_end(side.cuda_stream, C.byref(g))
                check(rc, "sdc_graph_end")
                ent["graph"] = g
            check(lib.sdc_graph_launch(ent["graph"], side.cuda_stream), "sdc_graph_launch")
            cur.wait_stream(side)
            return ent["eps"].clone()


class _LucidUNet(_HipUNet):
    ND = 2
    NORM_MODE = 0

    def __init__(self, dim, init_dim=None, out_dim=None, dim_mults=(1, 2, 4, 8), channels=3, self_condition=False,
                 resnet_block_groups=8, learned_variance=False, learned_sinusoidal_cond=False,
                 random_fourier_features=False, learned_sinusoidal_dim=16, sinusoidal_pos_emb_theta=10000,
                 attn_dim_head=32, attn_heads=4, condition_on_residual=None):
        unsupported = dict(init_dim=init_dim, out_dim=out_dim, self_condition=self_condition or None,
                           learned_variance=learned_variance or None,
                           learned_sinusoidal_cond=learned_sinusoidal_cond or None,
                           random_fourier_features=random_fourier_features or None,
                           condition_on_residual=condition_on_residual)
        bad = [k for k, v in unsupported.items() if v is not None]
        if bad or attn_dim_head != 32 or attn_heads != 4 or sinusoidal_pos_emb_theta != 10000:
            raise NotImplementedError(f"options never enabled by the reference configs are not built: {bad}")
        super().__init__(spec_lucid(dim, tuple(dim_mults), channels, self.ND), dim)
        self.channels, self.dim_mults, self.groups = channels, tuple(dim_mults), resnet_block_groups
        self.out_dim = channels
        self.random_or_learned_sinusoidal_cond = False

    def _lin_attn(self, b, prefix, x):
        plan, pool = b.plan, b.plan.pool
        B, C = x.shape[0], x.shape[1]
        n = x.numel() // (B * C)
        if self.fuse_linattn and C in (64, 128) and n % 64 == 0:
            return plan.linattn_block(x, b.V(f"{prefix}.fn.norm.g"), b.W(f"{prefix}.fn.fn.to_qkv.weight"),
                                      b.W(f"{prefix}.fn.fn.to_out.0.weight"), b.V(f"{prefix}.fn.fn.to_out.0.bias"),
                                      b.V(f"{prefix}.fn.fn.to_out.1.g"), B, 1, n, (C * n, n, 0), self.NORM_MODE, self.NORM_MODE)
        xn = plan.chan_norm(x, b.V(f"{prefix}.fn.norm.g"), self.NORM_MODE)
        qkv = b.conv(xn, f"{prefix}.fn.fn.to_qkv", bias=False)
        pool.put(xn)
        o = pool.get((B, HID, *x.shape[2:]))
        plan.linattn(qkv, HEADS, B, 1, n, (3 * HID * n, n, 0), o, (HID * n, n, 0))
        pool.put(qkv)
        y = b.conv(o, f"{prefix}.fn.fn.to_out.0")
        pool.put(o)
        plan.chan_norm(y, b.V(f"{prefix}.fn.fn.to_out.1.g"), self.NORM_MODE, residual=x, out=y)
        return y

    def _full_attn(self, b, prefix, x):
        plan, pool = b.plan, b.plan.pool
        B, C = x.shape[0], x.shape[1]
        n = x.numel() // (B * C)
        xn = plan.chan_norm(x, b.V(f"{prefix}.fn.norm.g"), self.NORM_MODE)
        qkv = b.conv(xn, f"{prefix}.fn.fn.to_qkv", bias=False)
        pool.put(xn)
        o = pool.get((B, HID, *x.shape[2:]))
        plan.attn(qkv, o, HEADS, B, 1, n, (3 * HID * n, n, 0, 1), (HID * n, n, 0, 1))
        pool.put(qkv)
        y = b.conv(o, f"{prefix}.fn.fn.to_out", residual=x)
        pool.put(o)
        return y

    def _build(self, b, x, eps):
        pool, G = b.plan.pool, self.groups
        nres = len(self.dim_mults)
        x5, e5 = as5(x), as5(eps)
        h = b.conv(x5, "init_conv")
        r = h
        hs = []
        for i in range(nres):
            p = f"downs.{i}"
            x1 = b.resnet(f"{p}.0", h, G)
            if h is not r:
                pool.put(h)
            hs.append(x1)
            x2 = b.resnet(f"{p}.1", x1, G)
            x3 = self._lin_attn(b, f"{p}.2", x2)
            pool.put(x2)
            hs.append(x3)
            h = self._down(b, f"{p}.3", x3, i == nres - 1)
        m = b.resnet("mid_block1", h, G)
        pool.put(h)
        a = self._full_attn(b, "mid_attn", m)
        pool.put(m)
        h = b.resnet("mid_block2", a, G)
        pool.put(a)
        for i in range(nres):
            p = f"ups.{i}"
            s = hs.pop()
            y1 = b.resnet(f"{p}.0", h, G, x1=s)
            pool.put(h), pool.put(s)
            s = hs.pop()
            y2 = b.resnet(f"{p}.1", y1, G, x1=s)
            pool.put(y1), pool.put(s)
            y3 = self._lin_attn(b, f"{p}.2", y2)
            pool.put(y2)
            h = self._up(b, f"{p}.3", y3, i == nres - 1)
            pool.put(y3)
        b.final_conv("final_res_block", "final_conv", h, G, r, e5)
        pool.put(h), pool.put(r)


class Unet2D(_LucidUNet):
    ND, NORM_MODE = 2, 0

    def _down(self, b, p, x, last):
        if last:
            return b.conv(x, p)
        return b.conv(x, f"{p}.1", kind="unshuffle", stride=(1, 2, 2), pad=(0, 0, 0))

    def _up(self, b, p, x, last):
        if last:
            return b.conv(x, p)
        if self.subpixel_upsample:
            return b.plan.upsample2_conv3(x, lambda p=p: self.P(f"{p}.1.weight"), b.V(f"{p}.1.bias"), self.P(f"{p}.1.weight").shape[0])
        return b.conv(x, f"{p}.1", up=(1, 2, 2))


class Unet1D(_LucidUNet):
    ND, NORM_MODE = 1, 1

    def __init__(self, dim, init_dim=None, out_dim=None, dim_mults=(1, 2, 4, 8), channels=12, **kw):
        super().__init__(dim, init_dim, out_dim, dim_mults, channels, **kw)

    def _down(self, b, p, x, last):
        if last:
            return b.conv(x, p)
        return b.conv(x, p, stride=(1, 1, 2), pad=(0, 0, 1))

    def _up(self, b, p, x, last):
        if last:
            return b.conv(x, p)
        return b.conv(x, f"{p}.1", up=(1, 1, 2))


def rel_pos_bias_table(weight, n, num_buckets=32, max_distance=32):
    q = torch.arange(n)
    rel = q[None, :] - q[:, None]
    m = -rel
    nb = num_buckets // 2
    ret = (m < 0).long() * nb
    m = m.abs()
    max_exact = nb // 2
    small = m < max_exact
    large = max_exact + (torch.log(m.float() / max_exact) / math.log(max_distance / max_exact) * (nb - max_exact)).long()
    large = torch.min(large, torch.full_like(large, nb - 1))
    bucket = (ret + torch.where(small, m, large)).to(weight.device)
    return weight[bucket].permute(2, 0, 1).contiguous()


class Unet3D_with_Conv3D(_HipUNet):

    def __init__(self, dim, cond_dim=None, out_dim=None, dim_mults=(1, 2, 4, 8), channels=6, attn_heads=4,
                 attn_dim_head=32, use_bert_text_cond=False, init_dim=None, init_kernel_size=7,
                 use_sparse_linear_attn=True, block_type="resnet", resnet_groups=8):
        if (cond_dim is not None or out_dim is not None or use_bert_text_cond or init_dim is not None
                or init_kernel_size != 7 or not use_sparse_linear_attn or attn_heads != 4 or attn_dim_head != 32):
            raise NotImplementedError("options never enabled by the reference's 2D scripts are not built")
        super().__init__(spec_smoke(dim, tuple(dim_mults), channels), dim)
        self.channels, self.dim_mults, self.groups = channels, tuple(dim_mults), resnet_groups
        self.has_cond = False
        shared = self.P("init_temporal_attn.fn.fn.fn.rotary_emb.freqs")
        shared.requires_grad_(False)
        for k, _ in self._spec:
            if k.endswith("rotary_emb.freqs"):
                m = self
                for name in k.split(".")[:-1]:
                    m = m._modules[name]
                m._parameters["freqs"] = shared

    def _attn_tables(self, b, F):
        plan = b.plan
        if not hasattr(plan, "_rot"):
            def rot():
                fr = self.P("init_temporal_attn.fn.fn.fn.rotary_emb.freqs").detach().float().cpu()
                ang = torch.arange(F, dtype=torch.float32)[:, None] * fr[None, :]
                return torch.stack((ang.cos(), ang.sin()), dim=-1).reshape(-1)
            plan._rot = plan.packed(rot)
            plan._bias = plan.packed(lambda: rel_pos_bias_table(
                self.P("time_rel_pos_bias.relative_attention_bias.weight").detach(), F).reshape(-1))
        return plan._rot, plan._bias

    def _temporal(self, b, prefix, x):
        plan, pool = b.plan, b.plan.pool
        B, C, F, H, W = x.shape
        hw = H * W
        rot, bias = self._attn_tables(b, F)
        if self.fuse_linattn and C == 64 and F == 32 and hw % 8 == 0 and x.is_contiguous():
            if plan.attn_f16:
                return plan.tattn_block(x, b.V(f"{prefix}.fn.norm.gamma"), lambda: self.P(f"{prefix}.fn.fn.fn.to_qkv.weight"),
                                        lambda: self.P(f"{prefix}.fn.fn.fn.to_out.weight"), rot, bias)
            return plan.tattn_block(x, b.V(f"{prefix}.fn.norm.gamma"), b.W(f"{prefix}.fn.fn.fn.to_qkv.weight"),
                                    b.W(f"{prefix}.fn.fn.fn.to_out.weight"), rot, bias)
        xn = plan.chan_norm(x, b.V(f"{prefix}.fn.norm.gamma"), 0)
        qkv = b.conv(xn, f"{prefix}.fn.fn.fn.to_qkv", bias=False)
        pool.put(xn)
        o = pool.get((B, HID, F, H, W))
        plan.attn(qkv, o, HEADS, B, hw, F, (3 * HID * F * hw, F * hw, 1, hw), (HID * F * hw, F * hw, 1, hw), rot, bias)
        pool.put(qkv)
        y = b.conv(o, f"{prefix}.fn.fn.fn.to_out", bias=False, residual=x)
        pool.put(o)
        return y

    def _la_fusable(self, shape):
        B, C, F, H, W = shape
        return self.fuse_linattn and C in (64, 128) and (H * W) % 64 == 0 and B * F < 65536

    def _resnet_then_spatial_linear(self, b, res_prefix, la_prefix, x, G):
        pool = b.plan.pool
        cout = self.P(f"{res_prefix}.block2.proj.weight").shape[0]
        if self.fuse_gn_into_linattn and self._la_fusable((x.shape[0], cout, *x.shape[2:])):
            g, gn, r = b.resnet(res_prefix, x, G, defer_gn=True)
            y = self._spatial_linear(b, la_prefix, g, gn=gn)
            if r is not None:
                pool.put(r)
            return y, g
        a = b.resnet(res_prefix, x, G)
        return self._spatial_linear(b, la_prefix, a), a

    def _spatial_linear(self, b, prefix, x, gn=None):
        plan, pool = b.plan, b.plan.pool
        B, C, F, H, W = x.shape
        hw = H * W
        if self._la_fusable(x.shape):
            return plan.linattn_block(x, b.V(f"{prefix}.fn.norm.gamma"), b.W(f"{prefix}.fn.fn.to_qkv.weight"),
                                      b.W(f"{prefix}.fn.fn.to_out.weight"), b.V(f"{prefix}.fn.fn.to_out.bias"), None,
                                      B, F, hw, (C * F * hw, F * hw, hw), 0, -1, gn=gn)
        assert gn is None
        xn = plan.chan_norm(x, b.V(f"{prefix}.fn.norm.gamma"), 0)
        qkv = b.conv(xn, f"{prefix}.fn.fn.to_qkv", bias=False)
        pool.put(xn)
        o = pool.get((B, HID, F, H, W))
        plan.linattn(qkv, HEADS, B, F, hw, (3 * HID * F * hw, F * hw, hw), o, (HID * F * hw, F * hw, hw))
        pool.put(qkv)
        y = b.conv(o, f"{prefix}.fn.fn.to_out", residual=x)
        pool.put(o)
        return y

    def _spatial_full(self, b, prefix, x):
        plan, pool = b.plan, b.plan.pool
        B, C, F, H, W = x.shape
        hw = H * W
        xn = plan.chan_norm(x, b.V(f"{prefix}.fn.norm.gamma"), 0)
        qkv = b.conv(xn, f"{prefix}.fn.fn.fn.to_qkv", bias=False)
        pool.put(xn)
        o = pool.get((B, HID, F, H, W))
        plan.attn(qkv, o, HEADS, B, F, hw, (3 * HID * F * hw, F * hw, hw, 1), (HID * F * hw, F * hw, hw, 1))
        pool.put(qkv)
        y = b.conv(o, f"{prefix}.fn.fn.fn.to_out", bias=False, residual=x)
        pool.put(o)
        return y

    def _build(self, b, x, eps):
        pool, G = b.plan.pool, self.groups
        nres = len(self.dim_mults)
        x5 = x.permute(0, 2, 1, 3, 4)
        e5 = eps.permute(0, 2, 1, 3, 4)
        h0 = b.conv(x5, "init_conv")
        h = self._temporal(b, "init_temporal_attn", h0)
        pool.put(h0)
        r = h
        hs = []
        for i in range(nres):
            p = f"downs.{i}"
            a1 = b.resnet(f"{p}.0", h, G)
            if h is not r:
                pool.put(h)
            a3, a2 = self._resnet_then_spatial_linear(b, f"{p}.1", f"{p}.2", a1, G)
            pool.put(a1)
            pool.put(a2)
            a4 = self._temporal(b, f"{p}.3", a3)
            pool.put(a3)
            hs.append(a4)
            h = a4
            if i < nres - 1:
                h = b.conv(a4, f"{p}.4", stride=(1, 2, 2), pad=(0, 1, 1))
        m1 = b.resnet("mid_block1", h, G)
        m2 = self._spatial_full(b, "mid_spatial_attn", m1)
        pool.put(m1)
        m3 = self._temporal(b, "mid_temporal_attn", m2)
        pool.put(m2)
        h = b.resnet("mid_block2", m3, G)
        pool.put(m3)
        for i in range(nres):
            p = f"ups.{i}"
            s = hs.pop()
            u1 = b.resnet(f"{p}.0", h, G, x1=s)
            pool.put(h), pool.put(s)
            u3, u2 = self._resnet_then_spatial_linear(b, f"{p}.1", f"{p}.2", u1, G)
            pool.put(u1)
            pool.put(u2)
            u4 = self._temporal(b, f"{p}.3", u3)
            pool.put(u3)
            h = u4
            if i < nres - 1:
                h = b.plan.conv_transpose_422(u4, lambda p=p: self.P(f"{p}.4.weight"), b.V(f"{p}.4.bias"),
                                              self.P(f"{p}.4.weight").shape[1])
                pool.put(u4)
        b.final_conv("final_conv.0", "final_conv.1", h, G, r, e5)
        pool.put(h), pool.put(r)
```

Measured before the change: 0.2895 trajectories/s.

## Add split-bf16 Winograd 3x3x3 conv kernel on matrix cores

Adds a new Winograd F(2x2) kernel for 3x3x3 convolutions. It splits the transformed inputs and weights into three bf16 parts (hi/mid/lo) so the fp32-accurate products can run on bf16 MFMA, and it fuses GroupNorm partial statistics into the epilogue. The kernel is enabled by default for the U-Net's non-residual 3x3x3 convs when precision is 4 or 5. This aims to cut the fp32 ALU cost of the dominant conv layers. In exchange it adds extra weight packing, heavy register and LDS use (one wave per EU), and the accuracy risk of a three-term bf16 split.

```diff
diff --git a/include/sdc.h b/include/sdc.h
--- a/include/sdc.h
+++ b/include/sdc.h
@@ -168,6 +168,12 @@
 size_t sdc_pack_gemm_x3_bytes(int Cout, int Cin, int kH, int kW);
 int sdc_pack_gemm_x3(const float* wp, void* out, int Cout, int Cin, int kH, int kW, void* stream);
 int sdc_conv_gemm_x3(const SdcConvDesc* d, const float* x, const void* wb, const float* bias, float* y, void* stream);
+
+int sdc_conv_wino3_x3_ok(const SdcConvDesc* d);
+size_t sdc_pack_wino3_x3_bytes(int Cout, int Cin);
+int sdc_pack_wino3_x3(const float* wp, void* out, int Cout, int Cin, void* stream);
+int sdc_conv_wino3_x3(const SdcConvDesc* d, const float* x, const float* x1, const void* wb, const float* bias, float* y,
+                      double* gn_parts, int gn_groups, void* stream);
 
 size_t sdc_gn_silu_bwd_floats(int B, int C, int G, int64_t S);
 int sdc_gn_silu_bwd(const float* h, const float* gy, const float* stats, const float* gamma, const float* beta,
diff --git a/safediffcon_amd/_lib.py b/safediffcon_amd/_lib.py
--- a/safediffcon_amd/_lib.py
+++ b/safediffcon_amd/_lib.py
@@ -122,6 +122,10 @@
     "sdc_pack_gemm_x3_bytes": (C.c_size_t, [C.c_int, C.c_int, C.c_int, C.c_int]),
     "sdc_pack_gemm_x3": (C.c_int, [_f32p, C.c_void_p, C.c_int, C.c_int, C.c_int, C.c_int, _stream]),
     "sdc_conv_gemm_x3": (C.c_int, [C.POINTER(SdcConvDesc), _f32p, C.c_void_p, _f32p, _f32p, _stream]),
+    "sdc_conv_wino3_x3_ok": (C.c_int, [C.POINTER(SdcConvDesc)]),
+    "sdc_pack_wino3_x3_bytes": (C.c_size_t, [C.c_int, C.c_int]),
+    "sdc_pack_wino3_x3": (C.c_int, [_f32p, C.c_void_p, C.c_int, C.c_int, _stream]),
+    "sdc_conv_wino3_x3": (C.c_int, [C.POINTER(SdcConvDesc), _f32p, _f32p, C.c_void_p, _f32p, _f32p, C.c_void_p, C.c_int, _stream]),
     "sdc_conv_wgrad_f16_bytes": (C.c_size_t, [C.POINTER(SdcWgradDesc)]),
     "sdc_conv_wgrad_f16": (C.c_int, [C.POINTER(SdcWgradDesc), _f32p, _f32p, C.c_void_p, _f32p, _f32p, C.c_void_p, C.c_size_t, _stream]),
     "sdc_conv_wgrad_describe": (C.c_int, [C.POINTER(SdcWgradDesc), C.c_char_p, C.c_size_t]),
diff --git a/safediffcon_amd/build.py b/safediffcon_amd/build.py
--- a/safediffcon_amd/build.py
+++ b/safediffcon_amd/build.py
@@ -5,7 +5,7 @@
 HERE = os.path.dirname(os.path.abspath(__file__))
 CSRC = os.path.join(HERE, "csrc")
 LIB = os.path.join(HERE, "libsdc_hip.so")
-SOURCES = ["sdc_api.hip", "sdc_conv.hip", "sdc_conv_wino.hip", "sdc_conv_f16.hip", "sdc_conv_stem_f16.hip", "sdc_conv_stem_x3.hip", "sdc_conv_gemm_x3.hip", "sdc_norm.hip", "sdc_attn.hip", "sdc_lablock.hip", "sdc_tablock.hip", "sdc_tablock_f16.hip", "sdc_step.hip", "sdc_solver.hip", "sdc_grad.hip", "sdc_wgrad_f16.hip", "sdc_attn_bwd.hip", "sdc_kstar.hip", "sdc_smoke.hip", "sdc_linear.hip", "sdc_optim.hip"]
+SOURCES = ["sdc_api.hip", "sdc_conv.hip", "sdc_conv_wino.hip", "sdc_conv_f16.hip", "sdc_conv_stem_f16.hip", "sdc_conv_stem_x3.hip", "sdc_conv_gemm_x3.hip", "sdc_conv_wino_x3.hip", "sdc_norm.hip", "sdc_attn.hip", "sdc_lablock.hip", "sdc_tablock.hip", "sdc_tablock_f16.hip", "sdc_step.hip", "sdc_solver.hip", "sdc_grad.hip", "sdc_wgrad_f16.hip", "sdc_attn_bwd.hip", "sdc_kstar.hip", "sdc_smoke.hip", "sdc_linear.hip", "sdc_optim.hip"]
 HEADERS = ["sdc_common.h", "sdc_conv.h", "sdc_conv_wino3s.inc", "sdc_conv_wino2s.inc", "sdc_conv_pw2.inc"]
 HIPCC = os.environ.get("HIPCC", "/opt/rocm/bin/hipcc")
 FLAGS = ["--offload-arch=gfx950", "-O3", "-fPIC", "-std=c++17", "-Wall", "-Wno-unused-function"]
diff --git a/safediffcon_amd/csrc/sdc_conv_wino_x3.hip b/safediffcon_amd/csrc/sdc_conv_wino_x3.hip
--- /dev/null
+++ b/safediffcon_amd/csrc/sdc_conv_wino_x3.hip
@@ -0,0 +1,560 @@
+#include "sdc_conv.h"
+
+using namespace sdcconv;
+
+namespace {
+
+typedef __bf16 bf16x8 __attribute__((ext_vector_type(8)));
+typedef __bf16 bf16x4 __attribute__((ext_vector_type(4)));
+typedef float w2f2 __attribute__((ext_vector_type(2)));
+typedef float nfloat4 __attribute__((ext_vector_type(4)));
+typedef float nfloat2 __attribute__((ext_vector_type(2)));
+
+__device__ __forceinline__ w2f2 pk_add2(w2f2 a, w2f2 b) { w2f2 r; asm("v_pk_add_f32 %0, %1, %2" : "=v"(r) : "v"(a), "v"(b)); return r; }
+__device__ __forceinline__ w2f2 pk_sub2(w2f2 a, w2f2 b) { w2f2 r; asm("v_pk_add_f32 %0, %1, %2 neg_lo:[0,1] neg_hi:[0,1]" : "=v"(r) : "v"(a), "v"(b)); return r; }
+__device__ __forceinline__ w2f2 pk_fma2(w2f2 a, w2f2 b, w2f2 c) { w2f2 r; asm("v_pk_fma_f32 %0, %1, %2, %3" : "=v"(r) : "v"(a), "v"(b), "v"(c)); return r; }
+__device__ __forceinline__ w2f2 pk_fms2(w2f2 a, w2f2 b, w2f2 c) { w2f2 r; asm("v_pk_fma_f32 %0, %1, %2, %3 neg_lo:[0,0,1] neg_hi:[0,0,1]" : "=v"(r) : "v"(a), "v"(b), "v"(c)); return r; }
+__device__ __forceinline__ w2f2 pk_fnma2(w2f2 a, w2f2 b, w2f2 c) { w2f2 r; asm("v_pk_fma_f32 %0, %1, %2, %3 neg_lo:[0,1,0] neg_hi:[0,1,0]" : "=v"(r) : "v"(a), "v"(b), "v"(c)); return r; }
+__device__ __forceinline__ w2f2 pk_sumdiff(w2f2 c) {
+    w2f2 r;
+    asm("v_pk_add_f32 %0, %1, %1 op_sel:[0,1] op_sel_hi:[1,0] neg_hi:[0,1]" : "=v"(r) : "v"(c));
+    return r;
+}
+__device__ __forceinline__ w2f2 pk_sumdiff_fwd(w2f2 c) {
+    w2f2 r;
+    asm("v_pk_add_f32 %0, %1, %1 op_sel:[0,1] op_sel_hi:[0,1] neg_hi:[0,1]" : "=v"(r) : "v"(c));
+    return r;
+}
+__device__ __forceinline__ w2f2 pk_addsub(w2f2 s, w2f2 a) { w2f2 r; asm("v_pk_add_f32 %0, %1, %2 neg_hi:[0,1]" : "=v"(r) : "v"(s), "v"(a)); return r; }
+__device__ __forceinline__ w2f2 pk_sqacc(w2f2 a, w2f2 c) { w2f2 r; asm("v_pk_fma_f32 %0, %1, %1, %2" : "=v"(r) : "v"(a), "v"(c)); return r; }
+__device__ __forceinline__ uint64_t lo64(float k) { return (uint64_t)__builtin_bit_cast(uint32_t, k); }
+__device__ __forceinline__ w2f2 pks_mul(w2f2 a, float k) { w2f2 r; asm("v_pk_mul_f32 %0, %1, %2 op_sel_hi:[1,0]" : "=v"(r) : "v"(a), "s"(lo64(k))); return r; }
+__device__ __forceinline__ w2f2 pks_fma(w2f2 a, float k, w2f2 c) { w2f2 r; asm("v_pk_fma_f32 %0, %1, %2, %3 op_sel_hi:[1,0,1]" : "=v"(r) : "v"(a), "s"(lo64(k)), "v"(c)); return r; }
+__device__ __forceinline__ float sub_prev2(float x, float b) {
+    float r;
+    asm("v_sub_f32_dpp %0, %1, %2 row_shr:2 row_mask:0xf bank_mask:0xf bound_ctrl:0" : "=v"(r) : "v"(x), "v"(b));
+    return r;
+}
+__device__ __forceinline__ float sub_next2(float a, float x) {
+    float r;
+    asm("v_subrev_f32_dpp %0, %1, %2 row_shl:2 row_mask:0xf bank_mask:0xf bound_ctrl:0" : "=v"(r) : "v"(x), "v"(a));
+    return r;
+}
+__device__ __forceinline__ double wave_sum8(const double (&v)[8], int lane) {
+    double w[4], u[2];
+    const bool b5 = lane & 32, b4 = lane & 16, b3 = lane & 8;
+#pragma unroll
+    for (int i = 0; i < 4; ++i) w[i] = (b5 ? v[4 + i] : v[i]) + __shfl_xor(b5 ? v[i] : v[4 + i], 32, 64);
+#pragma unroll
+    for (int i = 0; i < 2; ++i) u[i] = (b4 ? w[2 + i] : w[i]) + __shfl_xor(b4 ? w[i] : w[2 + i], 16, 64);
+    double t = (b3 ? u[1] : u[0]) + __shfl_xor(b3 ? u[0] : u[1], 8, 64);
+    t += __shfl_xor(t, 4, 64);
+    t += __shfl_xor(t, 2, 64);
+    t += __shfl_xor(t, 1, 64);
+    return t;
+}
+
+__device__ __forceinline__ uint32_t cvt_pk_bf16(float a, float b) {
+    typedef __bf16 bf16x2 __attribute__((ext_vector_type(2)));
+    return __builtin_bit_cast(uint32_t, __builtin_convertvector(w2f2{a, b}, bf16x2));
+}
+__device__ __forceinline__ float bf16_lo(uint32_t p) { return __builtin_bit_cast(float, p << 16); }
+__device__ __forceinline__ float bf16_hi(uint32_t p) { return __builtin_bit_cast(float, p & 0xFFFF0000u); }
+__device__ __forceinline__ void split3(float x, __bf16& h, __bf16& m, __bf16& l) {
+#pragma clang fp contract(off)
+    h = (__bf16)x;
+    const float r = x - (float)h;
+    m = (__bf16)r;
+    l = (__bf16)(r - (float)m);
+}
+
+constexpr int X3_BM = 64, X3_TILES = 64, X3_SK = 16;
+constexpr int X3_PC = 4 * 64 * X3_SK * 2;
+constexpr int X3_IMG = 3 * X3_PC;
+constexpr int X3_U = 0, X3_V = 2 * X3_IMG;
+constexpr int X3_SCR = 4 * X3_IMG;
+constexpr int X3_STASH = X3_SCR + 4 * 8 * 8;
+constexpr int X3_LDS = X3_STASH + 256 * 8 * 4;
+constexpr int X3_RUN = 4 * 64 * X3_SK;
+
+struct WinoX3Args {
+    SdcConvDesc d;
+    const float* x0;
+    const float* x1;
+    const __bf16* wb;
+    const float* bias;
+    float* y;
+    int Cin;
+    uint32_t plane_bytes;
+    double* gn_part;
+    int gn_G, gn_cpg, gn_nparts;
+};
+
+template <int OW, int DBG = 0>
+__global__ __launch_bounds__(256) __attribute__((amdgpu_waves_per_eu(1))) void conv_wg3_x3_kernel(const WinoX3Args a) {
+    static_assert(OW == 16, "rows of 16: one lane per tile and stage channel quad");
+    constexpr int BM = X3_BM, TW = OW / 2, LGW = 4;
+    typedef const __attribute__((address_space(1))) char* gchar_p;
+    typedef const __attribute__((address_space(1))) nfloat2* gfloat2_p;
+    typedef unsigned int u32x4 __attribute__((ext_vector_type(4)));
+    typedef const __attribute__((address_space(1))) u32x4* guint4_p;
+    typedef __attribute__((address_space(1))) char* gwchar_p;
+    typedef __attribute__((address_space(1))) nfloat2* gwfloat2_p;
+    extern __shared__ __attribute__((aligned(16))) char lds[];
+
+    const SdcConvDesc& d = a.d;
+    const int tid = threadIdx.x;
+    const int lane = tid & 63;
+    const int wave = SDC_UNIFORM(tid >> 6);
+    const int wm = wave >> 1, wn = wave & 1;
+    const int l31 = lane & 31, lh = lane >> 5;
+    const int MT = d.Cout / BM;
+    const int lb = xcd_tile(blockIdx.x, gridDim.x);
+    const int mt = lb % MT;
+    const int m0 = mt * BM;
+    const int tile0 = (lb / MT) * X3_TILES;
+    const int H2 = d.oH >> 1, D2 = d.oD >> 1;
+    int ob, od, hp0;
+    {
+        const int rp0 = tile0 >> (LGW - 1);
+        const int q = (int)(((float)rp0 + 0.5f) * (1.0f / (float)H2));
+        const int b = (int)(((float)q + 0.5f) * (1.0f / (float)D2));
+        hp0 = SDC_UNIFORM(rp0 - q * H2);
+        ob = SDC_UNIFORM(b);
+        od = SDC_UNIFORM(2 * (q - b * D2));
+    }
+    const bool two = d.Cin1 > 0;
+
+    const int pr = 2 * (lane >> 4) + (lane & 1), pc0 = 2 * ((lane & 15) >> 1);
+    const int hp = hp0 + pr;
+    const bool up_ok = hp > 0, dn_ok = 2 * hp + 2 < d.iH;
+    const w2f2 m0p = {up_ok ? 1.0f : 0.0f, up_ok ? 1.0f : 0.0f}, m3p = {dn_ok ? 1.0f : 0.0f, dn_ok ? 1.0f : 0.0f};
+    const uint32_t rsel0 = up_ok ? OW * 4 : 0, rsel3 = dn_ok ? 2 * OW * 4 : 0;
+    const uint32_t vp = (uint32_t)((2 * hp) * OW + pc0) * 4u;
+    const int ptile = pr * TW + (pc0 >> 1);
+    const int vpark = X3_V + ptile * 32 + (((wave >> 1) ^ ((ptile >> 3) & 1)) * 16) + (wave & 1) * 8;
+    const int afrag = X3_U + (wm * 32 + l31) * 32 + (lh ^ ((l31 >> 3) & 1)) * 16;
+    const int bfrag = X3_V + (wn * 32 + l31) * 32 + (lh ^ ((l31 >> 3) & 1)) * 16;
+    uint32_t uoff[6];
+#pragma unroll
+    for (int k = 0; k < 6; ++k) {
+        const int it = tid + 256 * k;
+        uoff[k] = (uint32_t)(it >> 9) * a.plane_bytes + (uint32_t)(it & 511) * 16u;
+    }
+
+    const int64_t xs1_0 = d.x0s[1], xs1_1 = d.x1s[1];
+    const int cin0 = d.Cin0, cin = a.Cin;
+    const int S1 = cin / X3_SK;
+    const float* const x0p = a.x0 + (int64_t)ob * d.x0s[0] + (int64_t)od * d.x0s[2];
+    const float* const x1p = two ? a.x1 + (int64_t)ob * d.x1s[0] + (int64_t)od * d.x1s[2] : x0p;
+    const int64_t xs2_0 = d.x0s[2], xs2_1 = two ? d.x1s[2] : d.x0s[2];
+    const uint32_t lo_u = (uint32_t)(-od) >> 31, hi_u = (uint32_t)(od + 2 - d.iD) >> 31;
+
+    w2f2 raw[4][2][4];
+    int s_jd = 0, s_ci = 0;
+    float mka = 0.f, mkb = 0.f;
+    const float *f_xa = x0p, *f_xb = x0p;
+    int64_t f_sc = 0;
+    uint32_t voff = vp, voff0 = vp - rsel0, voff3 = vp + rsel3;
+    auto fetch_raw_begin = [&]() __attribute__((always_inline)) {
+        const bool first = s_ci < cin0;
+        f_sc = first ? xs1_0 : xs1_1;
+        const int64_t xs2 = first ? xs2_0 : xs2_1;
+        const int cbase = (first ? s_ci : s_ci - cin0) + wave * 4;
+        const float* bsel = (first ? x0p : x1p) + (int64_t)cbase * f_sc;
+        const int jd_u = SDC_UNIFORM(s_jd);
+        const uint32_t j0 = (uint32_t)((jd_u ^ 2) - 1) >> 31, j2 = (uint32_t)((jd_u ^ 1) - 1) >> 31, j3 = (uint32_t)((jd_u ^ 3) - 1) >> 31;
+        const int da = -(int)(j0 & lo_u);
+        const int db = 1 + (int)j3 * (2 * (int)hi_u - 1);
+        mka = __builtin_bit_cast(float, (0x3F800000u & ((j0 & (lo_u ^ 1u)) - 1u)) | (j2 << 31));
+        mkb = __builtin_bit_cast(float, (0x3F800000u & ((j3 & (hi_u ^ 1u)) - 1u)) | ((j0 | (j3 & hi_u)) << 31));
+        f_xa = bsel + da * xs2;
+        f_xb = bsel + db * xs2;
+        const int nci = s_ci + X3_SK;
+        const bool wrap = nci >= cin;
+        s_ci = wrap ? 0 : nci;
+        s_jd = wrap ? ((s_jd + 1) & 3) : s_jd;
+    };
+    auto fetch_raw_rows = [&](int ch, int sl) __attribute__((always_inline)) {
+        const gchar_p rb = (gchar_p)uniform_ptr((sl ? f_xb : f_xa) + ch * f_sc);
+        asm volatile("" : "+v"(voff), "+v"(voff0), "+v"(voff3));
+        const nfloat2 v0 = *(gfloat2_p)(rb + voff0), v1 = *(gfloat2_p)(rb + voff), v2 = *(gfloat2_p)(rb + voff + OW * 4), v3 = *(gfloat2_p)(rb + voff3);
+        raw[ch][sl][0] = w2f2{v0.x, v0.y}; raw[ch][sl][1] = w2f2{v1.x, v1.y};
+        raw[ch][sl][2] = w2f2{v2.x, v2.y}; raw[ch][sl][3] = w2f2{v3.x, v3.y};
+    };
+    w2f2 hrow[4][4];
+    w2f2 ka0, kb0, ka3, kb3;
+    auto h_begin = [&](float ca, float cb) __attribute__((always_inline)) {
+        ka0 = pks_mul(m0p, ca); kb0 = pks_mul(m0p, cb); ka3 = pks_mul(m3p, ca); kb3 = pks_mul(m3p, cb);
+    };
+    auto h_transform = [&](int ch, float ca, float cb) __attribute__((always_inline)) {
+        const w2f2 e1 = pks_fma(raw[ch][1][1], cb, pks_mul(raw[ch][0][1], ca));
+        const w2f2 e2 = pks_fma(raw[ch][1][2], cb, pks_mul(raw[ch][0][2], ca));
+        hrow[ch][0] = pk_fma2(raw[ch][1][0], kb0, pk_fms2(raw[ch][0][0], ka0, e2));
+        hrow[ch][1] = pk_add2(e1, e2);
+        hrow[ch][2] = pk_sub2(e2, e1);
+        hrow[ch][3] = pk_fnma2(raw[ch][1][3], kb3, pk_fnma2(raw[ch][0][3], ka3, e1));
+    };
+    float px[4], pf[4];
+    uint32_t ph[2], pm[2], pl[2];
+    w2f2 sdv[4];
+    auto park_step = [&](int buf, int j, int xi, int k) __attribute__((always_inline)) {
+#pragma clang fp contract(off)
+        if (k == 0) {
+#pragma unroll
+            for (int ch = 0; ch < 4; ++ch) {
+                const w2f2 cc = hrow[ch][j];
+                if (xi == 0) px[ch] = sub_prev2(cc.y, cc.y);
+                else if (xi == 1) { sdv[ch] = pk_sumdiff(cc); px[ch] = sdv[ch].x; }
+                else if (xi == 2) px[ch] = sdv[ch].y;
+                else px[ch] = sub_next2(cc.x, cc.x);
+            }
+            ph[0] = cvt_pk_bf16(px[0], px[1]);
+            ph[1] = cvt_pk_bf16(px[2], px[3]);
+        } else if (k == 1) {
+            pf[0] = bf16_lo(ph[0]); pf[1] = bf16_hi(ph[0]); pf[2] = bf16_lo(ph[1]); pf[3] = bf16_hi(ph[1]);
+#pragma unroll
+            for (int i = 0; i < 4; ++i) px[i] = px[i] - pf[i];
+        } else if (k == 2) {
+            pm[0] = cvt_pk_bf16(px[0], px[1]);
+            pm[1] = cvt_pk_bf16(px[2], px[3]);
+            pf[0] = bf16_lo(pm[0]); pf[1] = bf16_hi(pm[0]); pf[2] = bf16_lo(pm[1]); pf[3] = bf16_hi(pm[1]);
+        } else if (k == 3) {
+#pragma unroll
+            for (int i = 0; i < 4; ++i) px[i] = px[i] - pf[i];
+            pl[0] = cvt_pk_bf16(px[0], px[1]);
+            pl[1] = cvt_pk_bf16(px[2], px[3]);
+        } else {
+            char* dst = lds + vpark + buf * X3_IMG + xi * 2048;
+            *reinterpret_cast<uint2*>(dst) = make_uint2(ph[0], ph[1]);
+            *reinterpret_cast<uint2*>(dst + X3_PC) = make_uint2(pm[0], pm[1]);
+            *reinterpret_cast<uint2*>(dst + 2 * X3_PC) = make_uint2(pl[0], pl[1]);
+        }
+    };
+    u32x4 ureg[2][6];
+    int u_p = 0, u_st = 0, u_j = 0;
+    gchar_p u_base = (gchar_p)uniform_ptr(reinterpret_cast<const float*>(a.wb));
+    auto fetch_u_begin = [&]() __attribute__((always_inline)) {
+        const int jdc = (0xC9 >> (2 * u_p)) & 3;
+        const int run = ((mt * 4 + jdc) * S1 + u_st) * 4 + u_j;
+        u_base = (gchar_p)uniform_ptr(reinterpret_cast<const float*>(a.wb + (int64_t)run * X3_RUN));
+        const bool wj = u_j == 3, ws = wj && u_st + 1 == S1;
+        u_j = (u_j + 1) & 3;
+        u_st = ws ? 0 : (wj ? u_st + 1 : u_st);
+        u_p = ws ? ((u_p + 1) & 3) : u_p;
+    };
+    auto fetch_u_item = [&](int set, int k) __attribute__((always_inline)) {
+        asm volatile("" : "+v"(uoff[k]));
+        ureg[set][k] = *(guint4_p)(u_base + uoff[k]);
+    };
+    auto park_u_item = [&](int buf, int k) __attribute__((always_inline)) {
+        *reinterpret_cast<u32x4*>(lds + X3_U + buf * X3_IMG + (tid + 256 * k) * 16) = ureg[buf][k];
+    };
+    bf16x8 fr[2][6];
+    auto read_frag = [&](int buf, int xi, int set, int p) __attribute__((always_inline)) {
+        fr[set][p] = *reinterpret_cast<const bf16x8*>(lds + (p < 3 ? afrag : bfrag) + buf * X3_IMG + (p % 3) * X3_PC + xi * 2048);
+    };
+
+    f32x16 acc[16];
+    f32x16 zero16, biasv;
+#pragma unroll
+    for (int r = 0; r < 16; ++r) { zero16[r] = 0.0f; biasv[r] = a.bias ? a.bias[m0 + wm * 32 + 8 * (r >> 2) + 4 * lh + (r & 3)] : 0.0f; }
+
+    float pka, pkb;
+    {
+        fetch_raw_begin();
+        pka = mka; pkb = mkb;
+#pragma unroll
+        for (int g = 0; g < 8; ++g) fetch_raw_rows(g >> 1, g & 1);
+        fetch_u_begin();
+#pragma unroll
+        for (int k = 0; k < 6; ++k) fetch_u_item(0, k);
+        fetch_u_begin();
+#pragma unroll
+        for (int k = 0; k < 6; ++k) fetch_u_item(1, k);
+        h_begin(pka, pkb);
+#pragma unroll
+        for (int ch = 0; ch < 4; ++ch) h_transform(ch, pka, pkb);
+#pragma unroll
+        for (int k = 0; k < 6; ++k) park_u_item(0, k);
+#pragma unroll
+        for (int st = 0; st < 20; ++st) park_step(0, 0, st / 5, st % 5);
+        fetch_u_begin();
+#pragma unroll
+        for (int k = 0; k < 6; ++k) fetch_u_item(0, k);
+    }
+    __syncthreads();
+#pragma unroll
+    for (int p = 0; p < 6; ++p) read_frag(0, 0, 0, p);
+
+    const int cob = m0 + wm * 32;
+    const int nloc = wn * 32 + l31;
+    const int ohp = hp0 + (nloc >> (LGW - 1)), otw = nloc & (TW - 1);
+    const uint32_t yoff = (uint32_t)((2 * ohp) * d.ys[3] + (2 * otw) * d.ys[4] + (4 * lh) * d.ys[1]) * 4u;
+    const uint32_t yoff1 = yoff + (uint32_t)d.ys[3] * 4u;
+    const bool gn = a.gn_part != nullptr;
+    float gp[8];
+    float* const gstash = reinterpret_cast<float*>(lds + X3_STASH) + tid * 8;
+
+    auto fold = [&](const int p) __attribute__((always_inline)) {
+        const bool t0 = p == 1 || p == 2, t1 = p != 2;
+        const bool ld0 = p == 2, ld1 = p == 1 || p == 3;
+        const bool fin0 = p == 2, fin1 = p == 3;
+        const bool always = d.Cout > 0;
+        const int LEAD = 2;
+        const int64_t ycs4 = d.ys[1] * 4;
+        float* const y0p = a.y + (int64_t)ob * d.ys[0] + (int64_t)od * d.ys[2] + (int64_t)cob * d.ys[1];
+        gwchar_p s0 = (gwchar_p)(__attribute__((address_space(1))) void*)uniform_ptr(y0p);
+        gwchar_p s1 = (gwchar_p)(__attribute__((address_space(1))) void*)uniform_ptr(y0p + d.ys[2]);
+        gchar_p l0 = (gchar_p)s0, l1 = (gchar_p)s1;
+        w2f2 P0[4][4][2], P1[4][4][2];
+        auto load_block = [&](int g4) __attribute__((always_inline)) {
+#pragma unroll
+            for (int r3 = 0; r3 < 4; ++r3) {
+                if (ld0) { P0[g4][r3][0] = *(gfloat2_p)(l0 + yoff); P0[g4][r3][1] = *(gfloat2_p)(l0 + yoff1); l0 += r3 < 3 ? ycs4 : 5 * ycs4; }
+                if (ld1) { P1[g4][r3][0] = *(gfloat2_p)(l1 + yoff); P1[g4][r3][1] = *(gfloat2_p)(l1 + yoff1); l1 += r3 < 3 ? ycs4 : 5 * ycs4; }
+            }
+        };
+        if (ld0 || ld1) {
+#pragma unroll
+            for (int g = 0; g < LEAD; ++g) load_block(g);
+        }
+#pragma unroll
+        for (int g4 = 0; g4 < 4; ++g4) {
+            if (g4 + LEAD < 4 && (ld0 || ld1)) load_block(g4 + LEAD);
+            if (!always) continue;
+            w2f2 bs2 = {0.f, 0.f}, bq2 = {0.f, 0.f};
+#pragma unroll
+            for (int r3 = 0; r3 < 4; ++r3) {
+                const int rr = g4 * 4 + r3;
+                w2f2 pa[4], pb[4];
+#pragma unroll
+                for (int j = 0; j < 4; ++j) {
+                    pa[j] = w2f2{acc[4 * j][rr], acc[4 * j + 3][rr]};
+                    pb[j] = w2f2{acc[4 * j + 1][rr], acc[4 * j + 2][rr]};
+                }
+                const w2f2 t0a = pk_add2(pk_add2(pa[0], pa[1]), pa[2]), t1a = pk_sub2(pk_sub2(pa[1], pa[2]), pa[3]);
+                const w2f2 t0b = pk_add2(pk_add2(pb[0], pb[1]), pb[2]), t1b = pk_sub2(pk_sub2(pb[1], pb[2]), pb[3]);
+                const w2f2 z0 = pk_addsub(pk_sumdiff_fwd(t0b), t0a);
+                const w2f2 z1 = pk_addsub(pk_sumdiff_fwd(t1b), t1a);
+                if (t0) {
+                    const bool have = p == 1 ? ld1 : ld0;
+                    const w2f2 b0 = p == 1 ? P1[g4][r3][0] : P0[g4][r3][0], b1 = p == 1 ? P1[g4][r3][1] : P0[g4][r3][1];
+                    const w2f2 u0 = have ? pk_add2(b0, z0) : z0, u1 = have ? pk_add2(b1, z1) : z1;
+                    *(gwfloat2_p)(s0 + yoff) = nfloat2{u0.x, u0.y};
+                    *(gwfloat2_p)(s0 + yoff1) = nfloat2{u1.x, u1.y};
+                    s0 += r3 < 3 ? ycs4 : 5 * ycs4;
+                    if (fin0) { bs2 = pk_add2(bs2, pk_add2(u0, u1)); bq2 = pk_sqacc(u1, pk_sqacc(u0, bq2)); }
+                }
+                if (t1) {
+                    const w2f2 u0 = ld1 ? pk_sub2(P1[g4][r3][0], z0) : z0, u1 = ld1 ? pk_sub2(P1[g4][r3][1], z1) : z1;
+                    *(gwfloat2_p)(s1 + yoff) = nfloat2{u0.x, u0.y};
+                    *(gwfloat2_p)(s1 + yoff1) = nfloat2{u1.x, u1.y};
+                    s1 += r3 < 3 ? ycs4 : 5 * ycs4;
+                    if (fin1) { bs2 = pk_add2(bs2, pk_add2(u0, u1)); bq2 = pk_sqacc(u1, pk_sqacc(u0, bq2)); }
+                }
+            }
+            if (fin0 || fin1) { gp[2 * g4] = bs2.x + bs2.y; gp[2 * g4 + 1] = bq2.x + bq2.y; }
+        }
+        if (fin0 && gn) {
+            *reinterpret_cast<nfloat4*>(gstash) = nfloat4{gp[0], gp[1], gp[2], gp[3]};
+            *reinterpret_cast<nfloat4*>(gstash + 4) = nfloat4{gp[4], gp[5], gp[6], gp[7]};
+        }
+    };
+
+    auto substage = [&](auto FIRST, auto J, const int pass) __attribute__((always_inline)) {
+        constexpr bool first = decltype(FIRST)::value;
+        constexpr int j = decltype(J)::value;
+        constexpr int rbuf = j & 1, wbuf = rbuf ^ 1, jn = (j + 1) & 3;
+        constexpr int PA[6] = {2, 1, 0, 1, 0, 0}, PB[6] = {0, 1, 2, 0, 1, 0};
+#pragma unroll
+        for (int sl = 0; sl < 24; ++sl) {
+            const int xi = sl / 6, t = sl % 6, c = 4 * j + xi, set = xi & 1;
+            const f32x16 cstart = (first && t == 0) ? ((c == 5 && pass == 0) ? biasv : zero16) : acc[c];
+            if (!(DBG & 64) || t == 0) acc[c] = __builtin_amdgcn_mfma_f32_32x32x16_bf16(fr[set][PA[t]], fr[set][3 + PB[t]], cstart, 0, 0, 0);
+            if (DBG & 16) {}
+            else if (xi < 3) read_frag(rbuf, xi + 1, set ^ 1, t);
+            else if (t >= 3) { read_frag(wbuf, 0, 0, 2 * (t - 3)); read_frag(wbuf, 0, 0, 2 * (t - 3) + 1); }
+            if (sl < 6) { if (!(DBG & 4)) park_u_item(wbuf, sl); }
+            else if (sl < 12) { if (sl == 6) fetch_u_begin(); if (!(DBG & 2)) fetch_u_item(wbuf, sl - 6); }
+            if (sl < 20 && !(DBG & 1)) park_step(wbuf, jn, sl / 5, sl % 5);
+            if (j == 0 && sl >= 12 && sl < 20 && !(DBG & 8)) {
+                if (sl == 12) { fetch_raw_begin(); pka = mka; pkb = mkb; }
+                fetch_raw_rows((sl - 12) >> 1, (sl - 12) & 1);
+            }
+            if (j == 2 && sl >= 20) {
+                if (sl == 20) h_begin(pka, pkb);
+                h_transform(sl - 20, pka, pkb);
+            }
+            __builtin_amdgcn_sched_barrier(0);
+            if (sl == 20 && !(DBG & 32)) __syncthreads();
+        }
+    };
+    auto stage = [&](auto FIRST, const int pass) __attribute__((always_inline)) {
+        substage(FIRST, std::integral_constant<int, 0>{}, pass);
+        substage(FIRST, std::integral_constant<int, 1>{}, pass);
+        substage(FIRST, std::integral_constant<int, 2>{}, pass);
+        substage(FIRST, std::integral_constant<int, 3>{}, pass);
+    };
+    auto run_pass = [&](auto P) __attribute__((always_inline)) {
+        constexpr int p = decltype(P)::value;
+        stage(std::true_type{}, p);
+        for (int st = 1; st < S1; ++st) stage(std::false_type{}, p);
+        fold(p);
+#pragma unroll
+        for (int q = 0; q < 6; ++q) read_frag(0, 0, 0, q);
+    };
+    run_pass(std::integral_constant<int, 0>{});
+    run_pass(std::integral_constant<int, 1>{});
+    run_pass(std::integral_constant<int, 2>{});
+    run_pass(std::integral_constant<int, 3>{});
+
+    if (gn) {
+        int tid = threadIdx.x;
+        asm volatile("" : "+v"(tid));
+        const int lane = tid & 63;
+        double* scr = reinterpret_cast<double*>(lds + X3_SCR);
+        double gv[8];
+        {
+            const nfloat4 s0 = *reinterpret_cast<const nfloat4*>(gstash), s1 = *reinterpret_cast<const nfloat4*>(gstash + 4);
+            const float g0[8] = {s0.x, s0.y, s0.z, s0.w, s1.x, s1.y, s1.z, s1.w};
+#pragma unroll
+            for (int i = 0; i < 8; ++i) gv[i] = (double)g0[i] + (double)gp[i];
+        }
+        const double tot = wave_sum8(gv, lane);
+        if ((lane & 7) == 0) scr[wave * 8 + (lane >> 3)] = tot;
+        __syncthreads();
+        const int ngl = a.gn_cpg >= BM ? 1 : BM / a.gn_cpg;
+        if (tid < ngl) {
+            const int r0 = a.gn_cpg >= BM ? 0 : tid * a.gn_cpg, r1 = a.gn_cpg >= BM ? BM : r0 + a.gn_cpg;
+            double sum = 0.0, sq = 0.0;
+            for (int blk = r0 / 8; blk < r1 / 8; ++blk) {
+                const int wmi = blk >> 2, k = blk & 3;
+                for (int wni = 0; wni < 2; ++wni) {
+                    sum += scr[((wmi * 2 + wni) * 4 + k) * 2];
+                    sq += scr[((wmi * 2 + wni) * 4 + k) * 2 + 1];
+                }
+            }
+            const int g = (m0 + r0) / a.gn_cpg;
+            const int ntl = tile0 / X3_TILES - ob * (D2 * H2 * TW / X3_TILES);
+            const int idx = a.gn_cpg >= BM ? ntl * (a.gn_cpg / BM) + (m0 - g * a.gn_cpg) / BM : ntl;
+            double* pp = a.gn_part + (((int64_t)ob * a.gn_G + g) * a.gn_nparts + idx) * 2;
+            pp[0] = sum; pp[1] = sq;
+        }
+    }
+}
+
+__global__ __launch_bounds__(256) void pack_wino3_x3_kernel(const float* __restrict__ u3, __bf16* __restrict__ out, int Cout, int Cin, int64_t n) {
+    const int64_t e = (int64_t)blockIdx.x * 256 + threadIdx.x;
+    if (e >= n) return;
+    const int c16 = (int)(e & 15), col = (int)((e >> 4) & 63), xi = (int)((e >> 10) & 3), j = (int)((e >> 12) & 3);
+    int64_t r = e >> 14;
+    const int S1 = Cin / 16;
+    const int st = (int)(r % S1); r /= S1;
+    const int jd = (int)(r & 3);
+    const int mt = (int)(r >> 2);
+    const int ci = st * 16 + (c16 ^ (((col >> 3) & 1) << 3)), co = mt * 64 + col;
+    __bf16 ph, pm, pl;
+    split3(u3[(((int64_t)jd * Cin + ci) * Cout + co) * 16 + j * 4 + xi], ph, pm, pl);
+    out[e] = ph; out[n + e] = pm; out[2 * n + e] = pl;
+}
+
+bool x3_small(const SdcConvDesc& d) {
+    auto span = [](const int64_t* st, int b, int dd, int h, int w) {
+        return (int64_t)(b - 1) * st[0] + (int64_t)(dd - 1) * st[2] + (int64_t)(h - 1) * st[3] + (int64_t)(w - 1) * st[4];
+    };
+    return span(d.x0s, d.B, d.iD, d.iH, d.iW) < (1ll << 30) && (d.Cin1 == 0 || span(d.x1s, d.B, d.iD, d.iH, d.iW) < (1ll << 30));
+}
+
+bool wino3_x3_covers(const SdcConvDesc& d) {
+    if (!(d.B > 0 && d.Cin0 > 0 && d.Cin1 >= 0 && d.Cout > 0 && d.oW == 16)) return false;
+    if (d.Cin0 % X3_SK != 0 || d.Cin1 % X3_SK != 0) return false;
+    SdcConvDesc e = d;
+    e.precision = 4;
+    if (!wg3_ok(e, x3_small(e))) return false;
+    return (int64_t)64 * (d.Cin0 + d.Cin1) * d.Cout * 2 < (1ll << 30);
+}
+
+int wino3_x3_gnparts(const SdcConvDesc& d, int G) {
+    if (G <= 0 || d.Cout % G) return 0;
+    const int cpg = d.Cout / G;
+    const int64_t S = (int64_t)d.oD * d.oH * d.oW;
+    const int bn = X3_TILES * 8;
+    if (cpg % 8 || S % bn || !(cpg % X3_BM == 0 || X3_BM % cpg == 0)) return 0;
+    return (int)(S / bn) * (cpg >= X3_BM ? cpg / X3_BM : 1);
+}
+
+bool wino3_x3_faster(const SdcConvDesc& d) {
+    if (!(d.oD == 32 && d.oH == 16 && d.oW == 16)) return false;
+    const int c0 = d.Cin0, c1 = d.Cin1, co = d.Cout;
+    return (c0 == 128 && c1 == 0 && co == 256) || (c0 == 256 && c1 == 0 && co == 256) || (c0 == 256 && c1 == 256 && co == 128);
+}
+
+}
+
+extern "C" int sdc_conv_wino3_x3_ok(const SdcConvDesc* dp) {
+    return dp && wino3_x3_covers(*dp) && wino3_x3_faster(*dp) ? 1 : 0;
+}
+
+extern "C" size_t sdc_pack_wino3_x3_bytes(int Cout, int Cin) {
+    if (Cout <= 0 || Cout % 64 != 0 || Cin <= 0 || Cin % 16 != 0) return 0;
+    return (size_t)3 * 64 * Cin * Cout * sizeof(__bf16);
+}
+
+extern "C" int sdc_pack_wino3_x3(const float* wp, void* out, int Cout, int Cin, void* stream) {
+    SDC_REQUIRE(wp && out, SDC_ENULL, "sdc_pack_wino3_x3: null pointer");
+    SDC_REQUIRE(sdc_pack_wino3_x3_bytes(Cout, Cin) > 0, SDC_EINVAL, "sdc_pack_wino3_x3: Cout a multiple of 64, Cin a multiple of 16 (got Cin %d, Cout %d)", Cin, Cout);
+    const int64_t n = (int64_t)64 * Cin * Cout;
+    SDC_REQUIRE(n / 256 + 1 < (1ll << 31), SDC_EINVAL, "sdc_pack_wino3_x3: weight too large");
+    const int64_t K = (int64_t)27 * Cin;
+    const float* u3 = wp + K * Cout + (K / 3 * 4) * Cout + (K / 9 * 16) * Cout;
+    hipLaunchKernelGGL(pack_wino3_x3_kernel, dim3((unsigned)((n + 255) / 256)), dim3(256), 0, sdc::as_stream(stream), u3,
+                       reinterpret_cast<__bf16*>(out), Cout, Cin, n);
+    return sdc::check_launch("sdc_pack_wino3_x3");
+}
+
+extern "C" int sdc_conv_wino3_x3(const SdcConvDesc* dp, const float* x, const float* x1, const void* wb, const float* bias, float* y,
+                                 double* gn_parts, int gn_groups, void* stream) {
+    SDC_REQUIRE(dp && x && wb && y, SDC_ENULL, "sdc_conv_wino3_x3: null pointer");
+    const SdcConvDesc& d = *dp;
+    SDC_REQUIRE(d.Cin1 <= 0 || x1, SDC_ENULL, "sdc_conv_wino3_x3: Cin1 > 0 but x1 is null");
+    SDC_REQUIRE(wino3_x3_covers(d), SDC_EINVAL, "sdc_conv_wino3_x3: descriptor not covered: %dx%dx%d taps, stride %dx%dx%d, Cin %d+%d, Cout %d, "
+                "residual %d, output %dx%dx%d", d.kD, d.kH, d.kW, d.sD, d.sH, d.sW, d.Cin0, d.Cin1, d.Cout, (int)(d.rs[1] != 0), d.oD, d.oH, d.oW);
+    auto al = [](const void* p, int b) { return reinterpret_cast<uintptr_t>(p) % b == 0; };
+    SDC_REQUIRE(al(wb, 16) && al(x, 8) && (d.Cin1 == 0 || al(x1, 8)) && al(y, 8), SDC_EALIGN,
+                "sdc_conv_wino3_x3: the packed weight buffer must be 16-byte aligned, x, x1 and y 8-byte aligned");
+    WinoX3Args a;
+    a.d = d;
+    a.x0 = x; a.x1 = x1; a.wb = reinterpret_cast<const __bf16*>(wb); a.bias = bias; a.y = y;
+    a.Cin = d.Cin0 + d.Cin1;
+    a.plane_bytes = (uint32_t)((int64_t)64 * a.Cin * d.Cout * 2);
+    a.gn_part = nullptr; a.gn_G = a.gn_cpg = a.gn_nparts = 0;
+    if (gn_parts) {
+        const int np = wino3_x3_gnparts(d, gn_groups);
+        SDC_REQUIRE(np > 0, SDC_EINVAL, "sdc_conv_wino3_x3: shape not covered by the fused statistics (%d groups over %d channels)", gn_groups, d.Cout);
+        a.gn_part = gn_parts; a.gn_G = gn_groups; a.gn_cpg = d.Cout / gn_groups; a.gn_nparts = np;
+    }
+    const int64_t tiles = (int64_t)d.B * (d.oD / 2) * (d.oH / 2) * (d.oW / 2);
+    const dim3 grid((unsigned)((tiles / X3_TILES) * (d.Cout / X3_BM)));
+#define X3_LAUNCH(D)                                                                                             \
+    do {                                                                                                         \
+        static std::atomic<uint64_t> attr{0};                                                                    \
+        SDC_LDS_OPTIN(attr, (conv_wg3_x3_kernel<16, D>), 160 * 1024, "sdc_conv_wino3_x3");                       \
+        hipLaunchKernelGGL((conv_wg3_x3_kernel<16, D>), grid, dim3(256), X3_LDS, sdc::as_stream(stream), a);     \
+    } while (0)
+#ifdef SDC_KERNEL_EXPERIMENTS
+    static const int dbg = exp_env("SDC_WG3X_DBG");
+    switch (dbg) {
+        case 0: break;
+        case 1: X3_LAUNCH(1); return sdc::check_launch("sdc_conv_wino3_x3"); case 2: X3_LAUNCH(2); return sdc::check_launch("sdc_conv_wino3_x3");
+        case 4: X3_LAUNCH(4); return sdc::check_launch("sdc_conv_wino3_x3"); case 8: X3_LAUNCH(8); return sdc::check_launch("sdc_conv_wino3_x3");
+        case 16: X3_LAUNCH(16); return sdc::check_launch("sdc_conv_wino3_x3"); case 32: X3_LAUNCH(32); return sdc::check_launch("sdc_conv_wino3_x3");
+        case 64: X3_LAUNCH(64); return sdc::check_launch("sdc_conv_wino3_x3"); case 6: X3_LAUNCH(6); return sdc::check_launch("sdc_conv_wino3_x3");
+        case 15: X3_LAUNCH(15); return sdc::check_launch("sdc_conv_wino3_x3"); case 31: X3_LAUNCH(31); return sdc::check_launch("sdc_conv_wino3_x3");
+        default: X3_LAUNCH(63); return sdc::check_launch("sdc_conv_wino3_x3");
+    }
+#endif
+    X3_LAUNCH(0);
+#undef X3_LAUNCH
+    return sdc::check_launch("sdc_conv_wino3_x3");
+}
diff --git a/safediffcon_amd/engine.py b/safediffcon_amd/engine.py
--- a/safediffcon_amd/engine.py
+++ b/safediffcon_amd/engine.py
@@ -145,6 +145,17 @@
     return torch.stack(split3_bf16(z)).reshape(-1).view(torch.float32)
 
 
+def pack_wino3_x3(wp4, cout, cin):
+    n = 64 * cin * cout
+    if cout <= 0 or cout % 64 or cin <= 0 or cin % 16 or wp4.dim() != 1 or wp4.numel() != (27 + 36 + 48 + 64) * cin * cout:
+        raise ValueError(f"pack_wino3_x3: Cout % 64 == 0, Cin % 16 == 0, the flat precision-4 buffer of a 3x3x3 conv "
+                         f"(got Cin {cin}, Cout {cout}, {tuple(wp4.shape)})")
+    u3 = wp4[-n:].to(torch.float32).reshape(4, cin // 16, 16, cout // 64, 64, 4, 4)
+    z = u3.permute(3, 0, 1, 5, 6, 4, 2).reshape(cout // 64, 4, cin // 16, 4, 4, 4, 2, 8, 2, 8)
+    z = torch.stack((z[:, :, :, :, :, :, 0], z[:, :, :, :, :, :, 1].flip(-2)), 6).contiguous()
+    return torch.stack(split3_bf16(z)).reshape(-1).view(torch.float32)
+
+
 def split3_bf16(x):
     h = x.bfloat16()
     r = x - h.float()
@@ -205,7 +216,7 @@
 
 class Plan:
 
-    def __init__(self, device, precision=0, stem_f16=False, stem_split=False, gemm_split=False, attn_f16=False):
+    def __init__(self, device, precision=0, stem_f16=False, stem_split=False, gemm_split=False, attn_f16=False, wino_split=False):
         self.device = torch.device(device)
         self.lib = _lib.get_lib()
         self.precision = int(precision)
@@ -214,6 +225,7 @@
         self.stem_f16 = bool(stem_f16)
         self.stem_split = bool(stem_split) and self.precision >= 4 and not self.stem_f16
         self.gemm_split = bool(gemm_split) and self.precision >= 4
+        self.wino_split = bool(wino_split) and self.precision in (4, 5)
         self.attn_f16 = bool(attn_f16)
         self.calls = []
         self.pool = Pool(self.device)
@@ -270,7 +282,7 @@
         return self.packed(lambda: (p() if callable(p) else p).reshape(-1))
 
     def conv(self, x, wp, bias, cout, k, *, x1=None, stride=(1, 1, 1), pad=(0, 0, 0), up=(1, 1, 1), up_mode=0,
-             residual=None, out=None, gn_groups=0, stem_w=None, gemm_w=None):
+             residual=None, out=None, gn_groups=0, stem_w=None, gemm_w=None, wino_w=None):
         B, c0, iD, iH, iW = x.shape
         c1 = 0 if x1 is None else x1.shape[1]
 
@@ -299,6 +311,20 @@
                 wb = self.packed(lambda: pack_gemm_x3(gemm_w(), cout, c0, k))
                 self.keep += [d, x, wb, bias, out]
                 self._emit(self.lib.sdc_conv_gemm_x3, C.byref(d), _ptr(x), _ptr(wb), _ptr(bias), _ptr(out))
+                return out
+        if self.wino_split and wino_w is not None and residual is None:
+            d = conv_desc(x, x1, out, None, cout, k, stride, pad, up, up_mode, 4)
+            if self.lib.sdc_conv_wino3_x3_ok(C.byref(d)) and not (self.split_small_grids and self.lib.sdc_conv_splitk_bytes(C.byref(d))):
+                wb = self.packed(lambda: pack_wino3_x3(wino_w(), cout, c0 + c1))
+                self.keep += [d, x, x1, wb, bias, out]
+                nparts = int(self.lib.sdc_conv_gnparts(C.byref(d), gn_groups)) if (gn_groups and self.fuse_gn_stats) else 0
+                parts = None
+                if nparts > 0:
+                    parts = torch.empty(B * gn_groups * nparts * 2, dtype=torch.float64, device=self.device)
+                    self.keep.append(parts)
+                    self._gn_parts[out.data_ptr()] = (parts, nparts, gn_groups)
+                self._emit(self.lib.sdc_conv_wino3_x3, C.byref(d), _ptr(x), _ptr(x1), _ptr(wb), _ptr(bias), _ptr(out), _ptr(parts),
+                           gn_groups if nparts > 0 else 0)
                 return out
         if callable(wp):
             wp = wp()
diff --git a/safediffcon_amd/unet.py b/safediffcon_amd/unet.py
--- a/safediffcon_amd/unet.py
+++ b/safediffcon_amd/unet.py
@@ -208,6 +208,9 @@
         if self.plan.gemm_split and kind == "conv" and k in ((1, 4, 4), (1, 1, 1)) and x1 is None and residual is None:
             return self.plan.conv(x, lambda: self.W(wkey, kind), b, cout, k, stride=stride, pad=pad, up=up, out=out, gn_groups=gn_groups,
                                   gemm_w=lambda: pack_conv_weight(self.net.P(wkey), kind, 0))
+        if self.plan.wino_split and kind == "conv" and k == (3, 3, 3) and residual is None:
+            return self.plan.conv(x, lambda: self.W(wkey, kind), b, cout, k, x1=x1, stride=stride, pad=pad, up=up, out=out,
+                                  gn_groups=gn_groups, wino_w=lambda: pack_conv_weight(self.net.P(wkey), kind, 4))
         return self.plan.conv(x, self.W(wkey, kind), b, cout, k, x1=x1, stride=stride, pad=pad, up=up,
                               up_mode=1 if kind == "convT" else 0, residual=residual, out=out, gn_groups=gn_groups)
 
@@ -272,6 +275,7 @@
         self.attn_f16 = False
         self.stem_split = True
         self.gemm_split = True
+        self.wino_split = True
         self.fuse_linattn = True
         self.fuse_gn_into_linattn = True
         self.content_stamp = True
@@ -394,7 +398,7 @@
     def entry(self, shape, rows, lut=False):
         key = (tuple(shape), rows, bool(lut), int(self.precision), bool(self.fuse_linattn), bool(self.subpixel_upsample),
                bool(self.fuse_gn_into_linattn), bool(self.split_small_grids), bool(self.fuse_final_conv), bool(self.stem_f16),
-               bool(self.stem_split), bool(self.gemm_split), bool(self.attn_f16))
+               bool(self.stem_split), bool(self.gemm_split), bool(self.attn_f16), bool(self.wino_split))
         stamp = self._weights_stamp()
         ent = self._plans.get(key)
         if ent is not None and ent["wstamp"] != stamp:
@@ -405,7 +409,7 @@
                 raise RuntimeError("safediffcon_amd runs on MI355X only: move the model to a cuda (HIP) device; "
                                    "there is no CPU fallback")
             plan = Plan(dev, precision=self.precision, stem_f16=bool(self.stem_f16), stem_split=bool(self.stem_split),
-                        gemm_split=bool(self.gemm_split), attn_f16=bool(self.attn_f16))
+                        gemm_split=bool(self.gemm_split), attn_f16=bool(self.attn_f16), wino_split=bool(self.wino_split))
             plan.split_small_grids = bool(self.split_small_grids)
             x = torch.zeros(shape, dtype=torch.float32, device=dev)
             eps = torch.zeros(shape, dtype=torch.float32, device=dev)
```

Result: faster. 0.2925 trajectories/s, median of 6 (+1.1%).
